# mengcaopku/DCNet

Measured on AMD Instinct MI355X. Metric: clips/sec (T=8, 416x416, bs8) fwd+bwd, higher is better.
Workload: dtype f32; 1 GPU; T=8 416x416 bs8/GPU L=20 fp32, 64 img/GPU/step as pairs, fwd+5 losses+bwd+RMSprop; arith=f16x2-split MFMA, fp32 accumulate, parallelism=dp1, ranks_seen=1, reducer=none, step=hipGraph replay (fwd+losses+bwd+RMSprop), sampler=mt

## Files before the change

dcnet_amd/csrc/coattn.h:

```cpp
#pragma once
#include <hip/hip_runtime.h>

int coattn_ld_pad(int hw);
bool coattn_on_gemm3(int b, int hw, int c);

struct CoOperand {
  const float* f; int ld; long long bs;
  const float* s; int lds; long long bss;
  const unsigned* amax;
};
inline CoOperand co_buffer(const float* p, int ld, long long bs, const unsigned* amax) { return CoOperand{p, ld, bs, p, ld, bs, amax}; }

struct CoProducts {
  int b, hw, c; hipStream_t stream; bool g3;
  CoProducts(int b_, int hw_, int c_, hipStream_t s) : b(b_), hw(hw_), c(c_), stream(s), g3(coattn_on_gemm3(b_, hw_, c_)) {}
  int nt(const CoOperand& A, const CoOperand& B, float* C, int ldc, long long c_bs, const float* row_scale, int accumulate,
         unsigned* amax_out = nullptr) const;
  int nn(const CoOperand& A, const CoOperand& B, float* C, int ldc, long long c_bs, const float* row_scale, int accumulate,
         unsigned* amax_out = nullptr) const;
  int tn(const CoOperand& A, const CoOperand& B, float* C, int ldc, long long c_bs, const float* row_scale, int accumulate,
         unsigned* amax_out = nullptr) const;
};

int coattn_amax_init_sets(unsigned* am, int sets, int slots, hipStream_t stream);
unsigned* coattn_ws_amax(float* ws, int b, int hw);
int coattn_amax_init(unsigned* am, hipStream_t stream);
int coattn_exp_sums(float* E, int nb, int hw, float temperature, float* rinv, float* cinv, float* ws, bool split, hipStream_t stream);
int coattn_rowdot_scale(const float* d, int ldd, long long bsd, const float* o, int ldo, long long bso, const float* inv, int b, int hw,
                        int c, float* delta, float* ds, unsigned* amax_d, unsigned* amax_ds, hipStream_t stream);
int coattn_da_bound(const unsigned* a1, const unsigned* a2, float temperature, unsigned* out, hipStream_t stream);
int coattn_dA(const float* E, float* dP1, const float* dP2, const float* rinv, const float* cinv, const float* d1, const float* d2,
              int b, int hw, float temperature, unsigned* amax_da, bool split, hipStream_t stream);
int coattn_fwd_operands(const CoOperand& F1, const CoOperand& F2, float* f1_attn, float* f2_attn, int ldo, long long bso, float* E,
                        float* rinv, float* cinv, float* ws, int b, int hw, int c, float temperature, hipStream_t stream);
```

dcnet_amd/csrc/coattn.hip:

```cpp
#include "igemm.h"
#include "prof.h"
#include "coattn.h"
#include "split4.h"

int tn_gemm_batched(const float* A, int lda, long long a_bs, const float* B, int ldb, long long b_bs,
                    float* C, int ldc, long long c_bs, const float* row_scale,
                    int M, int m_ld, int N, int K, int batch, int accumulate, hipStream_t stream,
                    const unsigned* amax_a = nullptr, const unsigned* amax_b = nullptr);

namespace {

constexpr int EXP_ROWS = 32;

template <bool SPLIT, bool COLS>
__global__ __launch_bounds__(256) void exp_sums_kernel(float* __restrict__ E, int hw, int ldE, float t,
                                                       float* __restrict__ rsum, float* __restrict__ colpart) {
  __shared__ float red[4][EXP_ROWS];
  const int b = blockIdx.y, rb = blockIdx.x;
  const int i0 = rb * EXP_ROWS;
  float* e = E + ((size_t)b * hw + i0) * ldE;
  float racc[EXP_ROWS];
#pragma unroll
  for (int r = 0; r < EXP_ROWS; ++r) racc[r] = 0.f;
  const int nrow = min(EXP_ROWS, hw - i0);
  for (int j = threadIdx.x * 4; j < ldE; j += 1024) {
    f32x4 v[EXP_ROWS];
#pragma unroll
    for (int r = 0; r < EXP_ROWS; ++r)
      v[r] = r < nrow ? *reinterpret_cast<const f32x4*>(e + (size_t)r * ldE + j) : f32x4{0.f, 0.f, 0.f, 0.f};
    f32x4 cs = {0.f, 0.f, 0.f, 0.f};
#pragma unroll
    for (int r = 0; r < EXP_ROWS; ++r) {
      if (r < nrow) {
        f32x4 o;
#pragma unroll
        for (int k = 0; k < 4; ++k) o[k] = (j + k < hw) ? expf(t * v[r][k] - t) : 0.f;
        if constexpr (SPLIT) split4_store(e + (size_t)r * ldE, j, o * SPLIT_SCALE_ONE);
        else *reinterpret_cast<f32x4*>(e + (size_t)r * ldE + j) = o;
        if constexpr (COLS) cs += o;
        racc[r] += (o[0] + o[1]) + (o[2] + o[3]);
      }
    }
    if constexpr (COLS) *reinterpret_cast<f32x4*>(colpart + ((size_t)rb * gridDim.y + b) * ldE + j) = cs;
  }
  const int lane = threadIdx.x & 63, wave = threadIdx.x >> 6;
#pragma unroll
  for (int r = 0; r < EXP_ROWS; ++r) {
    const float s = wave_sum(racc[r]);
    if (lane == 0) red[wave][r] = s;
  }
  __syncthreads();
  if (threadIdx.x < EXP_ROWS && i0 + threadIdx.x < hw)
    rsum[(size_t)b * hw + i0 + threadIdx.x] = 1.f / (red[0][threadIdx.x] + red[1][threadIdx.x] + red[2][threadIdx.x] + red[3][threadIdx.x]);
}

__global__ __launch_bounds__(256) void colsum_inv_kernel(const float* __restrict__ colpart, int nrb, int b, int hw, int ldE,
                                                         float* __restrict__ cinv) {
  const int j = blockIdx.x * 256 + threadIdx.x, bb = blockIdx.y;
  if (j >= hw) return;
  float s = 0.f;
  for (int rb = 0; rb < nrb; ++rb) s += colpart[((size_t)rb * b + bb) * ldE + j];
  cinv[(size_t)bb * hw + j] = 1.f / s;
}

enum { AM_ONE = 0, AM_DO1, AM_DO2, AM_DO1S, AM_DO2S, AM_DA, AM_DP1, AM_DP2, AM_SLOTS };
__global__ __launch_bounds__(256) void amax_init_kernel(unsigned* __restrict__ w, int total, int words_per_set) {
  for (int i = blockIdx.x * 256 + threadIdx.x; i < total; i += gridDim.x * 256)
    w[i] = (i % words_per_set) < DCN_AMAX_WORDS ? 0x3F800000u : 0u;
}

__global__ __launch_bounds__(256) void rowdot_scale_kernel(const float* __restrict__ d, int ldd, int64_t bsd,
                                                           const float* __restrict__ o, int ldo, int64_t bso, int hw,
                                                           const float* __restrict__ inv, int64_t rows, int c,
                                                           float* __restrict__ delta, float* __restrict__ ds,
                                                           unsigned* __restrict__ amax_d, unsigned* __restrict__ amax_ds) {
  __shared__ float red[4];
  const int lane = threadIdx.x & 63;
  const int64_t row = (int64_t)blockIdx.x * 4 + (threadIdx.x >> 6);
  float vmax = 0.f, s = 0.f;
  if (row < rows) {
    const int64_t bb = row / hw, i = row - bb * hw;
    s = inv[row];
    float acc = 0.f;
    for (int k = lane * 4; k < c; k += 256) {
      const f32x4 dv = *reinterpret_cast<const f32x4*>(d + bb * bsd + i * ldd + k);
      const f32x4 ov = *reinterpret_cast<const f32x4*>(o + bb * bso + i * ldo + k);
      acc += dv[0] * ov[0] + dv[1] * ov[1] + dv[2] * ov[2] + dv[3] * ov[3];
      *reinterpret_cast<f32x4*>(ds + row * c + k) = dv * s;
      vmax = fmaxf(fmaxf(vmax, fmaxf(fabsf(dv[0]), fabsf(dv[1]))), fmaxf(fabsf(dv[2]), fabsf(dv[3])));
    }
    acc = wave_sum(acc);
    if (lane == 0) delta[row] = acc;
  }
  const float vs = wave_max(vmax * s);
  amax_update_block(amax_d, vmax, red);
  __syncthreads();
  amax_update_block(amax_ds, vs, red);
}

template <bool ESPLIT, bool OSPLIT, bool COLS>
__global__ __launch_bounds__(256) void dA_kernel(const float* __restrict__ E, float* __restrict__ dP1, const float* __restrict__ dP2,
                                                 const float* __restrict__ rinv, const float* __restrict__ cinv,
                                                 const float* __restrict__ d1, const float* __restrict__ d2,
                                                 int hw, int ldE, float t, int64_t total4, unsigned* __restrict__ amax_da) {
  __shared__ float red[4];
  float vmax = 0.f;
  const int l4 = ldE >> 2;
  float s_out = 1.f;
  if constexpr (OSPLIT) s_out = split_pow2_scale(amax_read(amax_da));
  for (int64_t idx = (int64_t)blockIdx.x * 256 + threadIdx.x; idx < total4; idx += (int64_t)gridDim.x * 256) {
    const int64_t row = idx / l4;
    const int j = (int)(idx - row * l4) * 4;
    f32x4 e;
    if constexpr (ESPLIT) {
      const f32x4 hl = split4_load(E + row * ldE, j);
#pragma unroll
      for (int k = 0; k < 4; ++k) e[k] = hl[k] * (1.f / SPLIT_SCALE_ONE);
    } else {
      e = *reinterpret_cast<const f32x4*>(E + row * ldE + j);
    }
    const f32x4 p1 = *reinterpret_cast<const f32x4*>(dP1 + row * ldE + j);
    const float ri = rinv[row], di = d1[row];
    f32x4 o;
    if constexpr (COLS) {
      const int64_t bb = row / hw;
      const f32x4 p2 = *reinterpret_cast<const f32x4*>(dP2 + row * ldE + j);
#pragma unroll
      for (int k = 0; k < 4; ++k) {
        float v = 0.f;
        if (j + k < hw) v = t * e[k] * ((p1[k] - di) * ri + (p2[k] - d2[bb * hw + j + k]) * cinv[bb * hw + j + k]);
        o[k] = v;
      }
    } else {
      const float tr = t * ri;
#pragma unroll
      for (int k = 0; k < 4; ++k) o[k] = (j + k < hw) ? tr * e[k] * (p1[k] - di) : 0.f;
    }
    if constexpr (OSPLIT) {
      split4_store(dP1 + row * ldE, j, o * s_out);
    } else {
      *reinterpret_cast<f32x4*>(dP1 + row * ldE + j) = o;
      vmax = fmaxf(fmaxf(vmax, fmaxf(fabsf(o[0]), fabsf(o[1]))), fmaxf(fabsf(o[2]), fabsf(o[3])));
    }
  }
  if constexpr (!OSPLIT) amax_update_block(amax_da, vmax, red);
}

__global__ __launch_bounds__(64) void da_bound_kernel(const unsigned* __restrict__ a1, const unsigned* __restrict__ a2, float t,
                                                      unsigned* __restrict__ out) {
  const float b = 2.f * t * (__uint_as_float(amax_read(a1)) + (a2 ? __uint_as_float(amax_read(a2)) : 0.f));
  out[threadIdx.x & (DCN_AMAX_WORDS - 1)] = __float_as_uint(b);
}

inline int ld_pad(int hw) { return (hw + 31) / 32 * 32; }

void gemm_params(IgemmParams& p, const float* A, int lda, long long a_bs, const float* B, int ldb, long long b_bs,
                 float* C, int ldc, long long c_bs, int M, int N, int K, int batch) {
  p = IgemmParams{};
  p.osy = p.osx = p.isy = p.isx = 1; p.dense_out = 1;
  p.in = A; p.ldi = lda; p.in_bs = a_bs; p.wt = B; p.ldw = ldb; p.wt_bs = b_bs; p.out = C; p.ldo = ldc; p.out_bs = c_bs;
  p.ldr = ldc;
  p.N = 1; p.Hi = 1; p.Wi = M; p.Ho = 1; p.Wo = M; p.Hs = 1; p.Ws = M; p.M = M;
  p.Ci = K; p.Co = N; p.ntaps = 1; p.batch = batch;
}

}

static bool on_gemm3(int b, int hw, int c) { return c % 32 == 0 && gemm3_applicable(hw, c, hw, b) && gemm3_applicable(hw, hw, c, b); }

int coattn_ld_pad(int hw) { return ld_pad(hw); }
bool coattn_on_gemm3(int b, int hw, int c) { return on_gemm3(b, hw, c); }
unsigned* coattn_ws_amax(float* ws, int b, int hw) { return reinterpret_cast<unsigned*>(ws + (int64_t)cdiv(hw, EXP_ROWS) * b * ld_pad(hw)); }
int coattn_amax_init_sets(unsigned* am, int sets, int slots, hipStream_t stream) {
  const int total = sets * slots * DCN_AMAX_WORDS;
  hipLaunchKernelGGL(amax_init_kernel, dim3(cdiv(total, 256)), dim3(256), 0, stream, am, total, slots * DCN_AMAX_WORDS);
  DCN_CHECK_LAUNCH("coattn amax_init");
  return DCN_OK;
}
int coattn_amax_init(unsigned* am, hipStream_t stream) { return coattn_amax_init_sets(am, 1, AM_SLOTS, stream); }

int coattn_exp_sums(float* E, int nb, int hw, float temperature, float* rinv, float* cinv, float* ws, bool split, hipStream_t stream) {
  const int ldE = ld_pad(hw), nrb = cdiv(hw, EXP_ROWS);
  const auto kernel = split ? (cinv ? exp_sums_kernel<true, true> : exp_sums_kernel<true, false>)
                            : (cinv ? exp_sums_kernel<false, true> : exp_sums_kernel<false, false>);
  const int pid = prof_begin(12, (double)nb * hw * ldE * 8.0, stream);
  hipLaunchKernelGGL(kernel, dim3(nrb, nb), dim3(256), 0, stream, E, hw, ldE, temperature, rinv, ws);
  prof_end(pid, stream);
  DCN_CHECK_LAUNCH("exp_sums");
  if (!cinv) return DCN_OK;
  hipLaunchKernelGGL(colsum_inv_kernel, dim3(cdiv(hw, 256), nb), dim3(256), 0, stream, ws, nrb, nb, hw, ldE, cinv);
  DCN_CHECK_LAUNCH("colsum_inv");
  return DCN_OK;
}

int coattn_rowdot_scale(const float* d, int ldd, long long bsd, const float* o, int ldo, long long bso, const float* inv, int b, int hw,
                        int c, float* delta, float* ds, unsigned* amax_d, unsigned* amax_ds, hipStream_t stream) {
  const int64_t rows = (int64_t)b * hw;
  hipLaunchKernelGGL(rowdot_scale_kernel, dim3(cdiv(rows, 4)), dim3(256), 0, stream, d, ldd, (int64_t)bsd, o, ldo, (int64_t)bso, hw, inv, rows, c,
                     delta, ds, amax_d, amax_ds);
  DCN_CHECK_LAUNCH("rowdot_scale");
  return DCN_OK;
}

int coattn_da_bound(const unsigned* a1, const unsigned* a2, float temperature, unsigned* out, hipStream_t stream) {
  hipLaunchKernelGGL(da_bound_kernel, dim3(1), dim3(64), 0, stream, a1, a2, temperature, out);
  DCN_CHECK_LAUNCH("dA bound");
  return DCN_OK;
}

int coattn_dA(const float* E, float* dP1, const float* dP2, const float* rinv, const float* cinv, const float* d1, const float* d2,
              int b, int hw, float temperature, unsigned* amax_da, bool split, hipStream_t stream) {
  const int ldE = ld_pad(hw);
  const int64_t total4 = (int64_t)b * hw * (ldE / 4);
  int64_t g = (total4 + 255) / 256;
  if (g > 1024) g = 1024;
  const auto kernel = split ? (cinv ? dA_kernel<true, true, true> : dA_kernel<true, true, false>)
                            : (cinv ? dA_kernel<false, false, true> : dA_kernel<false, false, false>);
  const int pid = prof_begin(31, (double)total4 * 16.0 * (cinv ? 4.0 : 3.0), stream);
  hipLaunchKernelGGL(kernel, dim3((int)g), dim3(256), 0, stream, E, dP1, dP2, rinv, cinv, d1, d2, hw, ldE, temperature, total4, amax_da);
  prof_end(pid, stream);
  DCN_CHECK_LAUNCH("dA");
  return DCN_OK;
}

int CoProducts::nt(const CoOperand& A, const CoOperand& B, float* C, int ldc, long long c_bs, const float* row_scale, int accumulate,
                   unsigned* amax_out) const {
  if (g3) return gemm3_launch(A.s, A.lds, A.bss, 0, B.s, B.lds, B.bss, 0, C, ldc, c_bs, row_scale, row_scale ? hw : 0, hw, hw, c, b,
                              accumulate, A.amax, B.amax, stream, amax_out);
  IgemmParams p;
  gemm_params(p, A.f, A.ld, A.bs, B.f, B.ld, B.bs, C, ldc, c_bs, hw, hw, c, b);
  p.row_scale = row_scale; p.accumulate = accumulate; p.amax_a = A.amax; p.amax_b = B.amax;
  return igemm_launch(p, stream);
}
int CoProducts::nn(const CoOperand& A, const CoOperand& B, float* C, int ldc, long long c_bs, const float* row_scale, int accumulate,
                   unsigned* amax_out) const {
  if (g3) return gemm3_launch(A.s, A.lds, A.bss, 0, B.s, B.lds, B.bss, 1, C, ldc, c_bs, row_scale, row_scale ? hw : 0, hw, c, hw, b,
                              accumulate, A.amax, B.amax, stream, amax_out);
  IgemmParams p;
  gemm_params(p, A.f, A.ld, A.bs, B.f, B.ld, B.bs, C, ldc, c_bs, hw, c, A.ld, b);
  p.bmode = 1; p.kvalid = hw; p.row_scale = row_scale; p.accumulate = accumulate; p.amax_a = A.amax; p.amax_b = B.amax;
  return igemm_launch(p, stream);
}
int CoProducts::tn(const CoOperand& A, const CoOperand& B, float* C, int ldc, long long c_bs, const float* row_scale, int accumulate,
                   unsigned* amax_out) const {
  if (g3) return gemm3_launch(A.s, A.lds, A.bss, 1, B.s, B.lds, B.bss, 1, C, ldc, c_bs, row_scale, row_scale ? hw : 0, hw, c, hw, b,
                              accumulate, A.amax, B.amax, stream, amax_out);
  return tn_gemm_batched(A.f, A.ld, A.bs, B.f, B.ld, B.bs, C, ldc, c_bs, row_scale, hw, A.ld, c, hw, b, accumulate, stream, A.amax, B.amax);
}

int coattn_fwd_operands(const CoOperand& F1, const CoOperand& F2, float* f1_attn, float* f2_attn, int ldo, long long bso, float* E,
                        float* rinv, float* cinv, float* ws, int b, int hw, int c, float temperature, hipStream_t stream) {
  const CoProducts P(b, hw, c, stream);
  const int ldE = ld_pad(hw);
  const long long bsE = (long long)hw * ldE;
  const CoOperand Eo = co_buffer(E, ldE, bsE, F1.amax);
  int rc;
  if ((rc = P.nt(F1, F2, E, ldE, bsE, nullptr, 0))) return rc;
  if ((rc = coattn_exp_sums(E, b, hw, temperature, rinv, cinv, ws, P.g3, stream))) return rc;
  if ((rc = P.nn(Eo, F2, f1_attn, ldo, bso, rinv, 0))) return rc;
  if (f2_attn) rc = P.tn(Eo, F1, f2_attn, ldo, bso, cinv, 0);
  return rc;
}

extern "C" int64_t dcn_coattn_fwd_ws(int b, int hw, int c) {
  (void)c;
  return (int64_t)cdiv(hw, EXP_ROWS) * b * ld_pad(hw) + AM_SLOTS * DCN_AMAX_WORDS;
}
extern "C" int64_t dcn_coattn_e_size(int b, int hw) { return (int64_t)b * hw * ld_pad(hw); }
extern "C" int64_t dcn_coattn_saved_size(int b, int hw, int c) {
  return dcn_coattn_e_size(b, hw) + (on_gemm3(b, hw, c) ? (int64_t)2 * b * hw * c : 0);
}

extern "C" int dcn_coattn_fwd(const float* f1, const float* f2, int ldf, int64_t bsf, float* f1_attn, float* f2_attn, int ldo,
                              int64_t bso, float* E, float* rinv, float* cinv, float* ws,
                              int b, int hw, int c, float temperature, void* stream_) {
  hipStream_t stream = (hipStream_t)stream_;
  DCN_CHECK_ARG(f1 && f2 && f1_attn && E && rinv && cinv && ws, "coattn_fwd: null pointer");
  DCN_CHECK_ARG(b > 0 && hw > 0 && c > 0 && c % 32 == 0, "coattn_fwd: bad shape (c=%d must be a multiple of 32)", c);
  if (ldf <= 0) ldf = c;
  if (ldo <= 0) ldo = c;
  DCN_CHECK_ARG(ldf % 4 == 0 && ldo % 4 == 0, "coattn_fwd: ldf/ldo must be multiples of 4");
  if (bsf <= 0) bsf = (int64_t)hw * ldf;
  if (bso <= 0) bso = (int64_t)hw * ldo;
  DCN_CHECK_ARG(bsf % 4 == 0 && bso % 4 == 0, "coattn_fwd: batch strides must be multiples of 4");
  unsigned* am = coattn_ws_amax(ws, b, hw);
  int rc = coattn_amax_init(am, stream);
  if (rc) return rc;
  const unsigned* one = am + AM_ONE * DCN_AMAX_WORDS;
  float* f1s = E + dcn_coattn_e_size(b, hw);
  float* f2s = f1s + (int64_t)b * hw * c;
  const long long bss = (long long)hw * c;
  if (on_gemm3(b, hw, c)) {
    if ((rc = gemm3_presplit(f1, ldf, bsf, f1s, c, bss, b, hw, c, one, stream))) return rc;
    if ((rc = gemm3_presplit(f2, ldf, bsf, f2s, c, bss, b, hw, c, one, stream))) return rc;
  }
  return coattn_fwd_operands(CoOperand{f1, ldf, bsf, f1s, c, bss, one}, CoOperand{f2, ldf, bsf, f2s, c, bss, one}, f1_attn, f2_attn, ldo, bso,
                             E, rinv, cinv, ws, b, hw, c, temperature, stream);
}

extern "C" int64_t dcn_coattn_bwd_ws(int b, int hw, int c) {
  return (int64_t)2 * b * hw * ld_pad(hw) + (int64_t)2 * b * hw * c + (int64_t)2 * b * hw + AM_SLOTS * DCN_AMAX_WORDS +
         (on_gemm3(b, hw, c) ? (int64_t)2 * b * hw * c + 4 : 0);
}

extern "C" int dcn_coattn_bwd(const float* f1, const float* f2, int ldf, int64_t bsf,
                              const float* d_f1_attn, const float* d_f2_attn, int lddo, int64_t bsdo,
                              const float* f1_attn, const float* f2_attn, int ldo, int64_t bso,
                              const float* E, const float* rinv, const float* cinv,
                              float* d_f1, float* d_f2, int lddf, int64_t bsdf, int accumulate, float* ws,
                              int b, int hw, int c, float temperature, void* stream_) {
  hipStream_t stream = (hipStream_t)stream_;
  DCN_CHECK_ARG(f1 && f2 && d_f1_attn && d_f2_attn && f1_attn && f2_attn && E && rinv && cinv && d_f1 && d_f2 && ws,
                "coattn_bwd: null pointer");
  DCN_CHECK_ARG(b > 0 && hw > 0 && c > 0 && c % 32 == 0, "coattn_bwd: bad shape");
  if (ldf <= 0) ldf = c;
  if (ldo <= 0) ldo = c;
  if (lddo <= 0) lddo = c;
  if (lddf <= 0) lddf = c;
  if (bsf <= 0) bsf = (int64_t)hw * ldf;
  if (bso <= 0) bso = (int64_t)hw * ldo;
  if (bsdo <= 0) bsdo = (int64_t)hw * lddo;
  if (bsdf <= 0) bsdf = (int64_t)hw * lddf;
  const int ldE = ld_pad(hw);
  const long long rows = (long long)b * hw;
  float* dP1 = ws;
  float* dP2 = dP1 + rows * ldE;
  float* dO1s = dP2 + rows * ldE;
  float* dO2s = dO1s + rows * c;
  float* del1 = dO2s + rows * c;
  float* del2 = del1 + rows;
  unsigned* am = reinterpret_cast<unsigned*>(del2 + rows);
  int rc = coattn_amax_init(am, stream);
  if (rc) return rc;
  auto slot = [&](int i) { return am + i * DCN_AMAX_WORDS; };
  const CoProducts P(b, hw, c, stream);
  const long long bsE = (long long)hw * ldE, bss = (long long)hw * c;
  float* dO1p = reinterpret_cast<float*>(((uintptr_t)(am + AM_SLOTS * DCN_AMAX_WORDS) + 15) & ~(uintptr_t)15);
  float* dO2p = dO1p + rows * c;
  const float* f1s = E + dcn_coattn_e_size(b, hw);
  const float* f2s = f1s + rows * c;
  const CoOperand F1{f1, ldf, bsf, f1s, c, bss, slot(AM_ONE)}, F2{f2, ldf, bsf, f2s, c, bss, slot(AM_ONE)};
  const CoOperand DO1{d_f1_attn, lddo, bsdo, dO1p, c, bss, slot(AM_DO1)}, DO2{d_f2_attn, lddo, bsdo, dO2p, c, bss, slot(AM_DO2)};
  const CoOperand DO1S = co_buffer(dO1s, c, bss, slot(AM_DO1S)), DO2S = co_buffer(dO2s, c, bss, slot(AM_DO2S));
  const CoOperand Eo = co_buffer(E, ldE, bsE, slot(AM_ONE)), DA = co_buffer(dP1, ldE, bsE, slot(AM_DA));
  if ((rc = coattn_rowdot_scale(d_f1_attn, lddo, bsdo, f1_attn, ldo, bso, rinv, b, hw, c, del1, dO1s, slot(AM_DO1), slot(AM_DO1S), stream))) return rc;
  if ((rc = coattn_rowdot_scale(d_f2_attn, lddo, bsdo, f2_attn, ldo, bso, cinv, b, hw, c, del2, dO2s, slot(AM_DO2), slot(AM_DO2S), stream))) return rc;
  if (P.g3) {
    if ((rc = gemm3_presplit(d_f1_attn, lddo, bsdo, dO1p, c, bss, b, hw, c, slot(AM_DO1), stream))) return rc;
    if ((rc = gemm3_presplit(d_f2_attn, lddo, bsdo, dO2p, c, bss, b, hw, c, slot(AM_DO2), stream))) return rc;
    if ((rc = gemm3_presplit(dO1s, c, bss, dO1s, c, bss, b, hw, c, slot(AM_DO1S), stream))) return rc;
    if ((rc = gemm3_presplit(dO2s, c, bss, dO2s, c, bss, b, hw, c, slot(AM_DO2S), stream))) return rc;
  }
  if ((rc = P.nt(DO1, F2, dP1, ldE, bsE, nullptr, 0, slot(AM_DP1)))) return rc;
  if ((rc = P.nt(F1, DO2, dP2, ldE, bsE, nullptr, 0, slot(AM_DP2)))) return rc;
  if (P.g3 && (rc = coattn_da_bound(slot(AM_DP1), slot(AM_DP2), temperature, slot(AM_DA), stream))) return rc;
  if ((rc = coattn_dA(E, dP1, dP2, rinv, cinv, del1, del2, b, hw, temperature, slot(AM_DA), P.g3, stream))) return rc;
  if ((rc = P.nn(DA, F2, d_f1, lddf, bsdf, nullptr, accumulate))) return rc;
  if ((rc = P.nn(Eo, DO2S, d_f1, lddf, bsdf, nullptr, 1))) return rc;
  if ((rc = P.tn(DA, F1, d_f2, lddf, bsdf, nullptr, accumulate))) return rc;
  return P.tn(Eo, DO1S, d_f2, lddf, bsdf, nullptr, 1);
}
```

dcnet_amd/csrc/coattn_center.hip:

```cpp
#include "igemm.h"
#include "coattn.h"

namespace {

enum { AM_ONE = 0, AM_DO, AM_DOS, AM_DP, AM_DA, AM_SLOTS };

inline int frame_of(int n, int ctr) { return n < ctr ? n : n + 1; }

int check_shape(const char* who, int b, int t, int hw, int c, int ctr) {
  DCN_CHECK_ARG(b > 0 && hw > 0 && c > 0 && c % 32 == 0, "%s: bad shape (b=%d hw=%d; c=%d must be a multiple of 32)", who, b, hw, c);
  DCN_CHECK_ARG(t >= 2, "%s: a window needs t >= 2 frames (t=%d)", who, t);
  DCN_CHECK_ARG(ctr >= 0 && ctr < t, "%s: ctr=%d out of range [0, %d)", who, ctr, t);
  return DCN_OK;
}

}

extern "C" int64_t dcn_coattn_center_saved_size(int b, int t, int hw, int c) {
  if (b <= 0 || t < 2 || hw <= 0 || c <= 0) return 0;
  return dcn_coattn_e_size(b * (t - 1), hw) + (coattn_on_gemm3(b, hw, c) ? (int64_t)b * t * hw * c : 0);
}
extern "C" int64_t dcn_coattn_center_fwd_ws(int b, int t, int hw, int c) {
  (void)b; (void)t; (void)hw; (void)c;
  return AM_SLOTS * DCN_AMAX_WORDS;
}

extern "C" int dcn_coattn_center_fwd(const float* clips, float* attn, int ldo, int64_t bso, int64_t nso, float* E, float* rinv, float* ws,
                                     int b, int t, int hw, int c, int ctr, float temperature, void* stream_) {
  hipStream_t stream = (hipStream_t)stream_;
  DCN_CHECK_ARG(clips && attn && E && rinv && ws, "coattn_center_fwd: null pointer");
  int rc = check_shape("coattn_center_fwd", b, t, hw, c, ctr);
  if (rc) return rc;
  if (ldo <= 0) ldo = c;
  if (bso <= 0) bso = (int64_t)hw * ldo;
  if (nso <= 0) nso = (int64_t)b * bso;
  DCN_CHECK_ARG(ldo >= c && ldo % 4 == 0 && bso % 4 == 0 && nso % 4 == 0 && ((uintptr_t)attn & 15) == 0 && ((uintptr_t)clips & 15) == 0,
                "coattn_center_fwd: ldo >= c; ldo, the strides (floats) multiples of 4; 16-byte aligned tensors");
  const int ldE = coattn_ld_pad(hw), nn = t - 1;
  const long long bsE = (long long)hw * ldE, bsf = (long long)t * hw * c, frame = (long long)hw * c;
  const CoProducts P(b, hw, c, stream);
  unsigned* am = reinterpret_cast<unsigned*>(ws);
  if ((rc = coattn_amax_init_sets(am, 1, AM_SLOTS, stream))) return rc;
  const unsigned* one = am + AM_ONE * DCN_AMAX_WORDS;
  float* clips_s = E + dcn_coattn_e_size(b * nn, hw);
  auto frame_op = [&](int f) { return CoOperand{clips + f * frame, c, bsf, clips_s + f * frame, c, bsf, one}; };
  if (P.g3 && (rc = gemm3_presplit(clips, c, frame, clips_s, c, frame, b * t, hw, c, one, stream))) return rc;
  for (int n = 0; n < nn; ++n)
    if ((rc = P.nt(frame_op(ctr), frame_op(frame_of(n, ctr)), E + (int64_t)n * b * bsE, ldE, bsE, nullptr, 0))) return rc;
  if ((rc = coattn_exp_sums(E, b * nn, hw, temperature, rinv, nullptr, nullptr, P.g3, stream))) return rc;
  for (int n = 0; n < nn; ++n) {
    const CoOperand En = co_buffer(E + (int64_t)n * b * bsE, ldE, bsE, one);
    if ((rc = P.nn(En, frame_op(frame_of(n, ctr)), attn + n * nso, ldo, bso, rinv + (int64_t)n * b * hw, 0))) return rc;
  }
  return DCN_OK;
}

extern "C" int64_t dcn_coattn_center_bwd_ws(int b, int t, int hw, int c) {
  if (b <= 0 || t < 2 || hw <= 0 || c <= 0) return 0;
  const int64_t rows = (int64_t)b * hw;
  return rows * coattn_ld_pad(hw) + rows * c + rows + (int64_t)(t - 1) * AM_SLOTS * DCN_AMAX_WORDS + (coattn_on_gemm3(b, hw, c) ? rows * c + 4 : 0);
}

extern "C" int dcn_coattn_center_bwd(const float* clips, const float* d_attn, int lddo, int64_t bsdo, int64_t nsdo,
                                     const float* attn, int ldo, int64_t bso, int64_t nso, const float* E, const float* rinv,
                                     float* d_clips, int accumulate, float* ws,
                                     int b, int t, int hw, int c, int ctr, float temperature, void* stream_) {
  hipStream_t stream = (hipStream_t)stream_;
  DCN_CHECK_ARG(clips && d_attn && attn && E && rinv && d_clips && ws, "coattn_center_bwd: null pointer");
  int rc = check_shape("coattn_center_bwd", b, t, hw, c, ctr);
  if (rc) return rc;
  if (ldo <= 0) ldo = c;
  if (lddo <= 0) lddo = c;
  if (bso <= 0) bso = (int64_t)hw * ldo;
  if (bsdo <= 0) bsdo = (int64_t)hw * lddo;
  if (nso <= 0) nso = (int64_t)b * bso;
  if (nsdo <= 0) nsdo = (int64_t)b * bsdo;
  DCN_CHECK_ARG(ldo >= c && lddo >= c && ldo % 4 == 0 && lddo % 4 == 0 && bso % 4 == 0 && bsdo % 4 == 0 && nso % 4 == 0 && nsdo % 4 == 0 &&
                    (((uintptr_t)attn | (uintptr_t)d_attn | (uintptr_t)clips | (uintptr_t)d_clips | (uintptr_t)ws) & 15) == 0,
                "coattn_center_bwd: ldo, lddo >= c; row / batch / neighbour strides (floats) multiples of 4; 16-byte aligned tensors");
  const int ldE = coattn_ld_pad(hw), nn = t - 1;
  const long long rows = (long long)b * hw;
  const long long bsE = (long long)hw * ldE, bsf = (long long)t * hw * c, frame = (long long)hw * c;
  const CoProducts P(b, hw, c, stream);
  float* dP = ws;
  float* dOs = dP + rows * ldE;
  float* del = dOs + rows * c;
  unsigned* am = reinterpret_cast<unsigned*>(del + rows);
  float* dOp = reinterpret_cast<float*>(((uintptr_t)(am + (size_t)nn * AM_SLOTS * DCN_AMAX_WORDS) + 15) & ~(uintptr_t)15);
  if ((rc = coattn_amax_init_sets(am, nn, AM_SLOTS, stream))) return rc;
  const float* clips_s = E + dcn_coattn_e_size(b * nn, hw);
  for (int n = 0; n < nn; ++n) {
    const long long fj = frame_of(n, ctr) * frame, fc = ctr * frame;
    const float* rn = rinv + (int64_t)n * rows;
    const float* dO = d_attn + n * nsdo;
    unsigned* amn = am + (size_t)n * AM_SLOTS * DCN_AMAX_WORDS;
    auto slot = [&](int i) { return amn + i * DCN_AMAX_WORDS; };
    const CoOperand Fj{clips + fj, c, bsf, clips_s + fj, c, bsf, slot(AM_ONE)}, Fc{clips + fc, c, bsf, clips_s + fc, c, bsf, slot(AM_ONE)};
    const CoOperand DO{dO, lddo, bsdo, dOp, c, frame, slot(AM_DO)}, DOS = co_buffer(dOs, c, frame, slot(AM_DOS));
    const CoOperand En = co_buffer(E + (int64_t)n * b * bsE, ldE, bsE, slot(AM_ONE)), DA = co_buffer(dP, ldE, bsE, slot(AM_DA));
    if ((rc = coattn_rowdot_scale(dO, lddo, bsdo, attn + n * nso, ldo, bso, rn, b, hw, c, del, dOs, slot(AM_DO), slot(AM_DOS), stream))) return rc;
    if (P.g3) {
      if ((rc = gemm3_presplit(dO, lddo, bsdo, dOp, c, frame, b, hw, c, slot(AM_DO), stream))) return rc;
      if ((rc = gemm3_presplit(dOs, c, frame, dOs, c, frame, b, hw, c, slot(AM_DOS), stream))) return rc;
    }
    if ((rc = P.nt(DO, Fj, dP, ldE, bsE, nullptr, 0, slot(AM_DP)))) return rc;
    if (P.g3 && (rc = coattn_da_bound(slot(AM_DP), nullptr, temperature, slot(AM_DA), stream))) return rc;
    if ((rc = coattn_dA(En.f, dP, nullptr, rn, nullptr, del, nullptr, b, hw, temperature, slot(AM_DA), P.g3, stream))) return rc;
    if ((rc = P.nn(DA, Fj, d_clips + fc, c, bsf, nullptr, (n > 0 || accumulate) ? 1 : 0))) return rc;
    if ((rc = P.tn(DA, Fc, d_clips + fj, c, bsf, nullptr, 0))) return rc;
    if ((rc = P.tn(En, DOS, d_clips + fj, c, bsf, nullptr, 1))) return rc;
  }
  return DCN_OK;
}
```

dcnet_amd/csrc/gemm3.hip:

```cpp
#include "igemm.h"
#include "prof.h"
#include "split4.h"

namespace {

typedef _Float16 f16x8_t __attribute__((ext_vector_type(8)));
typedef short s16x4 __attribute__((ext_vector_type(4)));
typedef short s16x8 __attribute__((ext_vector_type(8)));
typedef __attribute__((address_space(3))) void lds_void;

#ifndef G3_ABL
#define G3_ABL 0
#endif
constexpr unsigned G3_OOB = 0x80000000u;
constexpr int G3_BM = 256, G3_BN = 256, G3_STAGES = 4;
constexpr int G3_TILE = 256 * 64;
constexpr int G3_STAGE = 2 * G3_TILE;
constexpr int G3_LDS = G3_STAGES * G3_STAGE;

struct G3Params {
  const float* A; const float* B; float* C;
  long long a_bs, b_bs, c_bs;
  int lda, ldb, ldc;
  int M, N, K;
  int a_rows, b_rows;
  int a_cols, b_cols;
  int tiles_m, tiles_n;
  const float* row_scale; long long rs_bs;
  int accumulate;
  const unsigned* amax_a; const unsigned* amax_b;
  unsigned* amax_out;
  int var;
  int abl;
};

__device__ __forceinline__ int g3_tswz(int krow) { return (krow & 1) | ((krow & 2) << 1); }

template <bool AT, bool BT, bool H1 = false>
__global__ __launch_bounds__(512, 1) void gemm3_kernel(const G3Params p) {
  extern __shared__ __attribute__((aligned(1024))) unsigned char smem3g[];
  const int tid = threadIdx.x, lane = tid & 63;
  const int wave = __builtin_amdgcn_readfirstlane(tid >> 6);
  const int wm = wave >> 2, wn = wave & 3;
  const int per_batch = p.tiles_m * p.tiles_n;
  const int lin = xcd_remap(blockIdx.x, gridDim.x);
  const int batch = __builtin_amdgcn_readfirstlane(lin / per_batch), t_ = lin - batch * per_batch;
  const int bm = __builtin_amdgcn_readfirstlane(t_ / p.tiles_n), bn = t_ - bm * p.tiles_n;
  const int m0 = bm * G3_BM, n0 = bn * G3_BN;
  const int kslices = (p.K + 15) >> 4;

  const float* a_base = p.A + batch * p.a_bs + (AT ? 0 : (long long)m0 * p.lda);
  const float* b_base = p.B + batch * p.b_bs + (BT ? 0 : (long long)n0 * p.ldb);
  const int a_rows_left = AT ? p.a_rows : p.a_rows - m0, b_rows_left = BT ? p.b_rows : p.b_rows - n0;
  const long long a_bytes = ((long long)(a_rows_left - 1) * p.lda + p.a_cols) * 4, b_bytes = ((long long)(b_rows_left - 1) * p.ldb + p.b_cols) * 4;
  const __amdgpu_buffer_rsrc_t a_rs = __builtin_amdgcn_make_buffer_rsrc((void*)a_base, 0, a_bytes > 0x7FFFFFF0LL ? 0x7FFFFFF0 : (int)a_bytes, 0x00020000);
  const __amdgpu_buffer_rsrc_t b_rs = __builtin_amdgcn_make_buffer_rsrc((void*)b_base, 0, b_bytes > 0x7FFFFFF0LL ? 0x7FFFFFF0 : (int)b_bytes, 0x00020000);

  unsigned voff[4];
  int sstep_a, sstep_b;
#pragma unroll
  for (int e = 0; e < 2; ++e) {
    const int j = 2 * wave + e;
    if (AT) {
      voff[e] = (unsigned)((long long)j * p.lda * 4 + m0 * 4 + ((lane ^ g3_tswz(j)) << 4));
      if (m0 + ((lane ^ g3_tswz(j)) << 2) >= p.a_cols) voff[e] = G3_OOB;
    } else {
      const int row = 16 * j + (lane >> 2), c = (lane & 3) ^ ((row >> 2) & 3);
      voff[e] = row < a_rows_left ? (unsigned)((long long)row * p.lda * 4 + c * 16) : G3_OOB;
    }
    if (BT) {
      voff[2 + e] = (unsigned)((long long)j * p.ldb * 4 + n0 * 4 + ((lane ^ g3_tswz(j)) << 4));
      if (n0 + ((lane ^ g3_tswz(j)) << 2) >= p.b_cols) voff[2 + e] = G3_OOB;
    } else {
      const int row = 16 * j + (lane >> 2), c = (lane & 3) ^ ((row >> 2) & 3);
      voff[2 + e] = row < b_rows_left ? (unsigned)((long long)row * p.ldb * 4 + c * 16) : G3_OOB;
    }
  }
  sstep_a = AT ? 16 * p.lda * 4 : 64;
  sstep_b = BT ? 16 * p.ldb * 4 : 64;
  const int my_dst = 2 * wave * 1024;

  int k_done = 0;
  auto issue_a = [&]() {
    const bool live = k_done < kslices && !(G3_ABL && (p.abl & 1));
    unsigned char* st = smem3g + (k_done & (G3_STAGES - 1)) * G3_STAGE + my_dst;
    int sa_ = live ? k_done * sstep_a : 0;
    if (G3_ABL && (p.abl & 8)) sa_ = 0;
#pragma unroll
    for (int e = 0; e < 2; ++e)
      __builtin_amdgcn_raw_ptr_buffer_load_lds(a_rs, (lds_void*)(st + e * 1024), 16, (int)(live ? voff[e] : G3_OOB), sa_, 0, 0);
  };
  auto issue_b = [&]() {
    const bool live = k_done < kslices && !(G3_ABL && (p.abl & 1));
    unsigned char* st = smem3g + (k_done & (G3_STAGES - 1)) * G3_STAGE + my_dst;
    int sb_ = live ? k_done * sstep_b : 0;
    if (G3_ABL && (p.abl & 8)) sb_ = 0;
#pragma unroll
    for (int e = 0; e < 2; ++e)
      __builtin_amdgcn_raw_ptr_buffer_load_lds(b_rs, (lds_void*)(st + G3_TILE + e * 1024), 16, (int)(live ? voff[2 + e] : G3_OOB), sb_, 0, 0);
    ++k_done;
  };
  auto issue = [&]() { issue_a(); issue_b(); };

  const int g = lane >> 5;
  const int hh = lane >> 5, gg = (lane >> 4) & 1, qq = (lane & 15) >> 2, pp = lane & 3;
  int a_rd[4][2], b_rd[2][2];
#pragma unroll
  for (int mi = 0; mi < 4; ++mi) {
    if (AT) {
      const int c = wm * 128 + mi * 32 + 16 * gg + 4 * pp;
#pragma unroll
      for (int r2 = 0; r2 < 2; ++r2) {
        const int kr = 8 * hh + 4 * r2 + qq;
        a_rd[mi][r2] = kr * 1024 + ((((c >> 3) * 2) ^ g3_tswz(kr)) << 4) + (c & 7) * 2;
      }
    } else {
      const int ar = wm * 128 + mi * 32 + (lane & 31);
      a_rd[mi][0] = ar * 64 + (((2 * g) ^ ((ar >> 2) & 3)) << 4);
      a_rd[mi][1] = ar * 64 + (((2 * g + 1) ^ ((ar >> 2) & 3)) << 4);
    }
  }
#pragma unroll
  for (int ni = 0; ni < 2; ++ni) {
    if (BT) {
      const int c = wn * 64 + ni * 32 + 16 * gg + 4 * pp;
#pragma unroll
      for (int r2 = 0; r2 < 2; ++r2) {
        const int kr = 8 * hh + 4 * r2 + qq;
        b_rd[ni][r2] = G3_TILE + kr * 1024 + ((((c >> 3) * 2) ^ g3_tswz(kr)) << 4) + (c & 7) * 2;
      }
    } else {
      const int br = wn * 64 + ni * 32 + (lane & 31);
      b_rd[ni][0] = G3_TILE + br * 64 + (((2 * g) ^ ((br >> 2) & 3)) << 4);
      b_rd[ni][1] = G3_TILE + br * 64 + (((2 * g + 1) ^ ((br >> 2) & 3)) << 4);
    }
  }
  auto tr_read = [&](const unsigned char* ptr) {
    return __builtin_amdgcn_ds_read_tr16_b64_v4i16((__attribute__((address_space(3))) s16x4*)(ptr));
  };
  auto tfrag = [&](const unsigned char* st, int off0, int off1, int plane) {
    const s16x4 lo = tr_read(st + (off0 ^ (plane << 4))), hi = tr_read(st + (off1 ^ (plane << 4)));
    const s16x8 v = {lo[0], lo[1], lo[2], lo[3], hi[0], hi[1], hi[2], hi[3]};
    return __builtin_bit_cast(f16x8_t, v);
  };

  f32x16 acc[4][2];
#pragma unroll
  for (int mi = 0; mi < 4; ++mi)
#pragma unroll
    for (int ni = 0; ni < 2; ++ni)
#pragma unroll
      for (int r = 0; r < 16; ++r) acc[mi][ni][r] = 0.f;

  for (int s = 0; s < G3_STAGES - 1; ++s) issue();

  asm volatile("s_waitcnt vmcnt(%0)" :: "n"((G3_STAGES - 2) * 4) : "memory");
  if (wm == 1) __builtin_amdgcn_s_barrier();
  for (int it = 0; it < kslices; ++it) {
    __builtin_amdgcn_s_barrier();
    asm volatile("" ::: "memory");
    const unsigned char* st = smem3g + (it & (G3_STAGES - 1)) * G3_STAGE;
    f16x8_t bh[2], bl[2];
    f16x8_t ah[4], al[4];
    if (G3_ABL && (p.abl & 2)) {
#pragma unroll
      for (int ni = 0; ni < 2; ++ni) { bh[ni] = f16x8_t{(_Float16)it, 0, 0, 0, 0, 0, 0, 0}; bl[ni] = bh[ni]; }
#pragma unroll
      for (int mi = 0; mi < 4; ++mi) { ah[mi] = bh[0]; al[mi] = bh[1]; }
    } else {
#pragma unroll
      for (int ni = 0; ni < 2; ++ni) {
        if (BT) { bh[ni] = tfrag(st, b_rd[ni][0], b_rd[ni][1], 0); if constexpr (!H1) bl[ni] = tfrag(st, b_rd[ni][0], b_rd[ni][1], 1); }
        else { bh[ni] = *reinterpret_cast<const f16x8_t*>(st + b_rd[ni][0]); if constexpr (!H1) bl[ni] = *reinterpret_cast<const f16x8_t*>(st + b_rd[ni][1]); }
      }
#pragma unroll
      for (int mi = 0; mi < 4; ++mi) {
        if (AT) { ah[mi] = tfrag(st, a_rd[mi][0], a_rd[mi][1], 0); if constexpr (!H1) al[mi] = tfrag(st, a_rd[mi][0], a_rd[mi][1], 1); }
        else { ah[mi] = *reinterpret_cast<const f16x8_t*>(st + a_rd[mi][0]); if constexpr (!H1) al[mi] = *reinterpret_cast<const f16x8_t*>(st + a_rd[mi][1]); }
      }
    }
    if (p.var >= 1) {
      issue_a();
      if (wm == 1) asm volatile("s_waitcnt vmcnt(%0)" :: "n"((G3_STAGES - 2) * 4 - 2) : "memory");
    } else {
      issue();
      if (wm == 1) asm volatile("s_waitcnt vmcnt(%0)" :: "n"((G3_STAGES - 2) * 4) : "memory");
    }
    asm volatile("s_waitcnt lgkmcnt(0)" ::: "memory");
    __builtin_amdgcn_s_barrier();
    asm volatile("" ::: "memory");
    if (G3_ABL && (p.abl & 4)) {
#pragma unroll
      for (int mi = 0; mi < 4; ++mi) { asm volatile("" :: "v"(ah[mi]), "v"(al[mi])); }
#pragma unroll
      for (int ni = 0; ni < 2; ++ni) { asm volatile("" :: "v"(bh[ni]), "v"(bl[ni])); }
    } else {
      __builtin_amdgcn_s_setprio(1);
      if constexpr (!H1) {
#pragma unroll
        for (int mi = 0; mi < 4; ++mi)
#pragma unroll
          for (int ni = 0; ni < 2; ++ni) acc[mi][ni] = __builtin_amdgcn_mfma_f32_32x32x16_f16(al[mi], bh[ni], acc[mi][ni], 0, 0, 0);
        if (p.var == 2) issue_b();
#pragma unroll
        for (int mi = 0; mi < 4; ++mi)
#pragma unroll
          for (int ni = 0; ni < 2; ++ni) acc[mi][ni] = __builtin_amdgcn_mfma_f32_32x32x16_f16(ah[mi], bl[ni], acc[mi][ni], 0, 0, 0);
      } else if (p.var == 2) issue_b();
#pragma unroll
      for (int mi = 0; mi < 4; ++mi)
#pragma unroll
        for (int ni = 0; ni < 2; ++ni) acc[mi][ni] = __builtin_amdgcn_mfma_f32_32x32x16_f16(ah[mi], bh[ni], acc[mi][ni], 0, 0, 0);
      __builtin_amdgcn_s_setprio(0);
    }
    if (p.var == 1) issue_b();
    if (wm == 0) asm volatile("s_waitcnt vmcnt(%0)" :: "n"((G3_STAGES - 2) * 4) : "memory");
  }
  if (wm == 0) __builtin_amdgcn_s_barrier();
  asm volatile("s_waitcnt vmcnt(0)" ::: "memory");

  const float dq = 1.f / (split_pow2_scale(amax_read(p.amax_a)) * split_pow2_scale(amax_read(p.amax_b)));
  float* __restrict__ cb = p.C + batch * p.c_bs;
  const float* rs = p.row_scale ? p.row_scale + batch * p.rs_bs : nullptr;
  float vmax = 0.f;
#pragma unroll
  for (int mi = 0; mi < 4; ++mi)
#pragma unroll
    for (int r = 0; r < 16; ++r) {
      const int m = m0 + wm * 128 + mi * 32 + 4 * g + (r & 3) + 8 * (r >> 2);
      if (m >= p.M) continue;
      const float f = rs ? dq * rs[m] : dq;
#pragma unroll
      for (int ni = 0; ni < 2; ++ni) {
        const int n = n0 + wn * 64 + ni * 32 + (lane & 31);
        if (n >= p.N) continue;
        float v = acc[mi][ni][r] * f;
        float* dst = cb + (long long)m * p.ldc + n;
        if (p.accumulate) v += *dst;
        *dst = v;
        vmax = fmaxf(vmax, fabsf(v));
      }
    }
  if (p.amax_out) {
    vmax = wave_max(vmax);
    if (lane == 0) amax_update(p.amax_out, vmax, blockIdx.x * 8 + wave);
  }
}

__global__ __launch_bounds__(256) void presplit_kernel(const float* __restrict__ src, int ld, long long bs, float* __restrict__ dst, int ldd,
                                                        long long bsd, int rows, int c, long long total8, const unsigned* __restrict__ amax) {
  const float s = split_pow2_scale(amax_read(amax));
  const int c8 = c >> 3;
  for (long long i = (long long)blockIdx.x * 256 + threadIdx.x; i < total8; i += (long long)gridDim.x * 256) {
    const long long row_all = i / c8; const int o = (int)(i - row_all * c8);
    const long long b = row_all / rows; const int row = (int)(row_all - b * rows);
    const float* sp = src + b * bs + (long long)row * ld + o * 8;
    const f32x4 x0 = *reinterpret_cast<const f32x4*>(sp) * s, x1 = *reinterpret_cast<const f32x4*>(sp + 4) * s;
    f16x8_t h, l;
#pragma unroll
    for (int e = 0; e < 4; ++e) { h[e] = (_Float16)x0[e]; h[4 + e] = (_Float16)x1[e]; }
#pragma unroll
    for (int e = 0; e < 4; ++e) { l[e] = (_Float16)(x0[e] - (float)h[e]); l[4 + e] = (_Float16)(x1[e] - (float)h[4 + e]); }
    float* dp = dst + b * bsd + (long long)row * ldd + o * 8;
    *reinterpret_cast<f16x8_t*>(dp) = h;
    *reinterpret_cast<f16x8_t*>(dp + 4) = l;
  }
}

DCN_KNOB(g_gemm3, "Gemm3", 1, "gemm3.hip: the co-attention products on pre-split operands (0 = implicit-GEMM / weight-gradient tiles; + 256 * v = schedule variant v; + 16 * bits = timing ablations, results WRONG)",
         nullptr, "-DG3_ABL=1", G3_ABL != 0, [](int v) { return (v & 0xF0) != 0; });
DCN_KNOB(g_gemm3_h1, "H1gemm3", 1, "gemm3.hip: one f16 piece per operand in the bf16 precision modes (0 = both pieces, fp32-accurate co-attention)");

template <bool AT, bool BT, bool H1>
int launch3g_(const G3Params& p, int grid, hipStream_t stream) {
  static DcnPerDeviceFlag attr_once;
  if (attr_once.first()) {
    (void)hipFuncSetAttribute(reinterpret_cast<const void*>(&gemm3_kernel<AT, BT, H1>), hipFuncAttributeMaxDynamicSharedMemorySize, G3_LDS);
  }
  hipLaunchKernelGGL((gemm3_kernel<AT, BT, H1>), dim3(grid), dim3(512), G3_LDS, stream, p);
  return DCN_OK;
}
template <bool AT, bool BT>
int launch3g(const G3Params& p, int grid, hipStream_t stream) {
  if (g_gemm3_h1 && igemm_precision() == 2) return launch3g_<AT, BT, true>(p, grid, stream);
  return launch3g_<AT, BT, false>(p, grid, stream);
}

}

int gemm3_variant() { const int v = g_gemm3 >> 8; return (v == 1 || v == 2) ? v : 0; }
extern "C" int dcn_gemm3_variant() { return gemm3_variant(); }

bool gemm3_applicable(int M, int N, int K, int batch) {
  return g_gemm3 && (igemm_precision() == 4 || igemm_precision() == 2) && M >= 512 && N >= 256 && K >= 64 && batch >= 1;
}

int gemm3_presplit(const float* src, int ld, long long bs, float* dst, int ldd, long long bsd, int batch, int rows, int c,
                   const unsigned* amax, hipStream_t stream) {
  DCN_CHECK_ARG(src && dst && amax && c % 8 == 0 && ld % 4 == 0 && ldd % 4 == 0 && bs % 4 == 0 && bsd % 4 == 0, "gemm3_presplit: bad argument");
  const long long total8 = (long long)batch * rows * (c / 8);
  long long g = (total8 + 255) / 256; if (g > 16384) g = 16384;
  hipLaunchKernelGGL(presplit_kernel, dim3((int)g), dim3(256), 0, stream, src, ld, bs, dst, ldd, bsd, rows, c, total8, amax);
  DCN_CHECK_LAUNCH("gemm3_presplit");
  return DCN_OK;
}

int gemm3_launch(const float* A, int lda, long long a_bs, int at, const float* B, int ldb, long long b_bs, int bt,
                 float* C, int ldc, long long c_bs, const float* row_scale, long long rs_bs,
                 int M, int N, int K, int batch, int accumulate, const unsigned* amax_a, const unsigned* amax_b, hipStream_t stream,
                 unsigned* amax_out) {
  DCN_CHECK_ARG(A && B && C && amax_a && amax_b, "gemm3: null pointer");
  DCN_CHECK_ARG(lda % 4 == 0 && ldb % 4 == 0 && a_bs % 4 == 0 && b_bs % 4 == 0 && (((uintptr_t)A | (uintptr_t)B) & 15) == 0, "gemm3: 16-byte rows");
  G3Params p{};
  p.A = A; p.B = B; p.C = C; p.a_bs = a_bs; p.b_bs = b_bs; p.c_bs = c_bs; p.lda = lda; p.ldb = ldb; p.ldc = ldc;
  p.M = M; p.N = N; p.K = K;
  const int k16 = (K + 15) / 16 * 16;
  p.a_rows = at ? K : M; p.b_rows = bt ? K : N;
  p.a_cols = at ? (M + 7) / 8 * 8 : k16; p.b_cols = bt ? (N + 7) / 8 * 8 : k16;
  DCN_CHECK_ARG(p.a_cols <= lda && p.b_cols <= ldb, "gemm3: rows shorter than the tile reads (lda=%d ldb=%d)", lda, ldb);
  p.tiles_m = cdiv(M, G3_BM); p.tiles_n = cdiv(N, G3_BN);
  p.row_scale = row_scale; p.rs_bs = rs_bs; p.accumulate = accumulate; p.amax_a = amax_a; p.amax_b = amax_b; p.amax_out = amax_out; p.abl = (g_gemm3 >> 4) & 15; p.var = gemm3_variant();
  const int grid = p.tiles_m * p.tiles_n * batch;
  const int pid = prof_begin(40, 2.0 * batch * (double)M * N * K, stream);
  int rc;
  if (at) rc = bt ? launch3g<true, true>(p, grid, stream) : DCN_ERR_ARG;
  else rc = bt ? launch3g<false, true>(p, grid, stream) : launch3g<false, false>(p, grid, stream);
  prof_end(pid, stream);
  DCN_CHECK_ARG(rc == DCN_OK, "gemm3: no A^T . B^T form");
  DCN_CHECK_LAUNCH("gemm3");
  return DCN_OK;
}

extern "C" int dcn_gemm3_supported(int m, int n, int k, int batch) { return gemm3_applicable(m, n, k, batch) ? 1 : 0; }

extern "C" int dcn_gemm3_presplit(const float* src, int ld, int64_t bs, float* dst, int ldd, int64_t bsd, int batch, int rows, int c,
                                  const uint32_t* amax, void* stream) {
  return gemm3_presplit(src, ld, bs, dst, ldd, bsd, batch, rows, c, amax, (hipStream_t)stream);
}

extern "C" int dcn_gemm3(const float* a, int lda, int64_t a_bs, int a_t, const float* b, int ldb, int64_t b_bs, int b_t,
                         float* c, int ldc, int64_t c_bs, const float* row_scale, int64_t rs_bs,
                         int m, int n, int k, int batch, int accumulate, const uint32_t* amax_a, const uint32_t* amax_b, void* stream) {
  DCN_CHECK_ARG(m > 0 && n > 0 && k > 0 && batch > 0, "gemm3: empty problem");
  return gemm3_launch(a, lda, a_bs, a_t, b, ldb, b_bs, b_t, c, ldc, c_bs, row_scale, rs_bs, m, n, k, batch, accumulate, amax_a, amax_b,
                      (hipStream_t)stream, nullptr);
}
```

dcnet_amd/csrc/igemm.h:

```cpp
#pragma once
#include "common.h"

#define IGEMM_MAX_TAPS 16


struct IgemmParams {
  const float* in;
  const float* wt;
  const float* f8;
  const unsigned* amax_a;
  const unsigned* amax_b;
  const void* wt16;
  const float* b_scale;
  unsigned* amax_out;
  float* out;
  const float* scale;
  const float* shift;
  const float* residual;
  float* stats;
  const float* row_scale;
  int batch;
  long long in_bs, wt_bs, out_bs;
  int bmode;
  int kvalid;
  int N, Hi, Wi, Ci, ldi;
  int Ho, Wo;
  int Hs, Ws;
  int oy0, ox0, osy, osx;
  int isy, isx;
  int Co, ldo, ldr, ldw;
  int M;
  int ntaps;
  int cpt, kiters;
  int act; float slope;
  int accumulate, dense_out, c4;
  int acc_post;
  int tap_dy[IGEMM_MAX_TAPS], tap_dx[IGEMM_MAX_TAPS], tap_w[IGEMM_MAX_TAPS];
  int ncls;
  int cls_M[4], cls_Hs[4], cls_Ws[4], cls_oy0[4], cls_ox0[4], cls_ntaps[4];
  const float* bt_y; const float* bt_mean; const float* bt_invstd; const float* bt_gamma; const float* bt_beta;
  int bt_act; float bt_slope;
  const unsigned char* a_scale8; const unsigned char* b_scale8;
};
inline double epilogue_reads(const IgemmParams& p) { return 1.0 + (p.accumulate ? 1.0 : 0.0) + (p.residual ? 1.0 : 0.0) + (p.bt_y ? 1.0 : 0.0); }
bool igemm_tap_capable(const IgemmParams& p);

int igemm_grid_m(int M, int Co, int ntaps);
int igemm_launch(const IgemmParams& p, hipStream_t stream);
bool igemm_will_presplit(long long rows, int Co, int ntaps, int Ci);

bool conv3_applicable(const IgemmParams& p, int precision, int gran);
int conv3_launch(const IgemmParams& p, int gran, hipStream_t stream);
bool conv3x_takes(const IgemmParams& p, int gran);
int conv3x_launch(const IgemmParams& p, int gran, hipStream_t stream);
int conv3b_bm(int M, int Co, int Wi);
bool conv3b_takes(const IgemmParams& p);
int conv3b_launch(const IgemmParams& p, int out_f32, hipStream_t stream);

bool conv1_applicable(const IgemmParams& p, int precision, int gran);
int conv1_launch(const IgemmParams& p, int gran, hipStream_t stream);
int conv1_tile_of(long long rows, int Co, int ntaps, int Ci, int stats, int gran, int storage16);
int conv1b_grid_m(int M, int Co, int ntaps, int s1_w = 0);
int conv1b_launch(const IgemmParams& p, int out_f32, hipStream_t stream);
int conv1q_grid_m(int M, int Co);
int conv1q_launch(const IgemmParams& p, int out_f32, hipStream_t stream);
bool conv2b_takes(int M, int Co, int ntaps);
int conv2b_launch(const IgemmParams& p, int out_f32, hipStream_t stream);


bool stem_applicable(const IgemmParams& p, const float* scratch);
int stem_launch(const IgemmParams& p, float* scratch, hipStream_t stream);

bool dgrad2_applicable(int n, int h, int wd, int cin, int cout, int ksize, int stride, int accumulate);
struct DcnBnTap { const float* y; const float* mean; const float* invstd; const float* gamma; const float* beta; int act; float slope;
                  float* stats; int stats_rows; };
int nconv1_launch_b16(int mode, const void* x, int ldi, const void* w16, void* y, int ldo, float* stats, int stats_rows,
                      int n, int h, int wd, int stride, hipStream_t stream);
int dgrad2_launch_b16(const void* dy, int lddy, const void* wt16, void* dx, int n, int h, int wd, int cin, int accumulate, hipStream_t stream);
int dgrad2_grid(int n, int h, int wd, int cin);
int dgrad2_launch(const float* dy, int lddy, const float* wt, float* dx, int n, int h, int wd, int cin, int accumulate,
                  const uint32_t* amax_dy, const uint32_t* amax_w, const DcnBnTap* tap, hipStream_t stream);
bool gemm3_applicable(int M, int N, int K, int batch);
int gemm3_presplit(const float* src, int ld, long long bs, float* dst, int ldd, long long bsd, int batch, int rows, int c,
                   const unsigned* amax, hipStream_t stream);
int gemm3_launch(const float* A, int lda, long long a_bs, int at, const float* B, int ldb, long long b_bs, int bt,
                 float* C, int ldc, long long c_bs, const float* row_scale, long long rs_bs,
                 int M, int N, int K, int batch, int accumulate, const unsigned* amax_a, const unsigned* amax_b, hipStream_t stream,
                 unsigned* amax_out = nullptr);
int igemm_precision();
extern int g_abl;
extern int g_wsplit;
struct DcnPreAct { const float* scale; const float* shift; int act; float slope; };
bool nconv1_applicable(int mode, int n, int h, int wd, int cin, int cout, int ksize, int stride);
int nconv1_launch(int mode, const float* x, int ldi, const float* w, float* y, int ldo, float* stats, int stats_rows,
                  int n, int h, int wd, int stride, const uint32_t* amax_x, const uint32_t* amax_w, const DcnPreAct* pre, hipStream_t stream);
```

Baseline: 88.12 clips/s.

## Fuse co-attention exp/softmax sums and dA into gemm3 product epilogues

Adds fused epilogues to the gemm3 co-attention kernel. In the forward pass the exponentials and per-tile row/column partial sums are computed inside the NT product, so the separate exp_sums pass over E is gone. In the backward pass the dA computation is done in the epilogue of the second dP product, which removes the dP2 buffer round trip and the standalone dA kernel; a norm of dO2 bounds the split scale in place of dP2's amax. The costs are heavier epilogues (LDS reductions, extra loads of E, rinv, cinv and the deltas), swapped MFMA operand order, a norm-based scale bound that may be looser, and small colsum kernels.

```diff
diff --git a/dcnet_amd/csrc/coattn.h b/dcnet_amd/csrc/coattn.h
--- a/dcnet_amd/csrc/coattn.h
+++ b/dcnet_amd/csrc/coattn.h
@@ -13,21 +13,26 @@
 
 struct CoProducts {
   int b, hw, c; hipStream_t stream; bool g3;
-  CoProducts(int b_, int hw_, int c_, hipStream_t s) : b(b_), hw(hw_), c(c_), stream(s), g3(coattn_on_gemm3(b_, hw_, c_)) {}
+  bool fused;
+  CoProducts(int b_, int hw_, int c_, hipStream_t s);
   int nt(const CoOperand& A, const CoOperand& B, float* C, int ldc, long long c_bs, const float* row_scale, int accumulate,
          unsigned* amax_out = nullptr) const;
   int nn(const CoOperand& A, const CoOperand& B, float* C, int ldc, long long c_bs, const float* row_scale, int accumulate,
          unsigned* amax_out = nullptr) const;
   int tn(const CoOperand& A, const CoOperand& B, float* C, int ldc, long long c_bs, const float* row_scale, int accumulate,
          unsigned* amax_out = nullptr) const;
+  int nt_exp(const CoOperand& A, const CoOperand& B, float* E, float temperature, float* rinv, float* cinv, float* ws) const;
+  int nt_dA(const CoOperand& A, const CoOperand& B, float* dP1, const float* E, const float* rinv, const float* cinv, const float* d1,
+            const float* d2, float temperature, const unsigned* amax_da) const;
 };
+int64_t coattn_exp_ws(int b, int hw, bool cols);
 
 int coattn_amax_init_sets(unsigned* am, int sets, int slots, hipStream_t stream);
 unsigned* coattn_ws_amax(float* ws, int b, int hw);
 int coattn_amax_init(unsigned* am, hipStream_t stream);
 int coattn_exp_sums(float* E, int nb, int hw, float temperature, float* rinv, float* cinv, float* ws, bool split, hipStream_t stream);
 int coattn_rowdot_scale(const float* d, int ldd, long long bsd, const float* o, int ldo, long long bso, const float* inv, int b, int hw,
-                        int c, float* delta, float* ds, unsigned* amax_d, unsigned* amax_ds, hipStream_t stream);
+                        int c, float* delta, float* ds, unsigned* amax_d, unsigned* amax_ds, hipStream_t stream, unsigned* norm_d = nullptr);
 int coattn_da_bound(const unsigned* a1, const unsigned* a2, float temperature, unsigned* out, hipStream_t stream);
 int coattn_dA(const float* E, float* dP1, const float* dP2, const float* rinv, const float* cinv, const float* d1, const float* d2,
               int b, int hw, float temperature, unsigned* amax_da, bool split, hipStream_t stream);
diff --git a/dcnet_amd/csrc/coattn.hip b/dcnet_amd/csrc/coattn.hip
--- a/dcnet_amd/csrc/coattn.hip
+++ b/dcnet_amd/csrc/coattn.hip
@@ -63,21 +63,23 @@
   cinv[(size_t)bb * hw + j] = 1.f / s;
 }
 
-enum { AM_ONE = 0, AM_DO1, AM_DO2, AM_DO1S, AM_DO2S, AM_DA, AM_DP1, AM_DP2, AM_SLOTS };
+enum { AM_ONE = 0, AM_DO1, AM_DO2, AM_DO1S, AM_DO2S, AM_DA, AM_DP1, AM_DP2, AM_NDO2, AM_SLOTS };
 __global__ __launch_bounds__(256) void amax_init_kernel(unsigned* __restrict__ w, int total, int words_per_set) {
   for (int i = blockIdx.x * 256 + threadIdx.x; i < total; i += gridDim.x * 256)
     w[i] = (i % words_per_set) < DCN_AMAX_WORDS ? 0x3F800000u : 0u;
 }
 
+template <bool NORM>
 __global__ __launch_bounds__(256) void rowdot_scale_kernel(const float* __restrict__ d, int ldd, int64_t bsd,
                                                            const float* __restrict__ o, int ldo, int64_t bso, int hw,
                                                            const float* __restrict__ inv, int64_t rows, int c,
                                                            float* __restrict__ delta, float* __restrict__ ds,
-                                                           unsigned* __restrict__ amax_d, unsigned* __restrict__ amax_ds) {
+                                                           unsigned* __restrict__ amax_d, unsigned* __restrict__ amax_ds,
+                                                           unsigned* __restrict__ norm_d) {
   __shared__ float red[4];
   const int lane = threadIdx.x & 63;
   const int64_t row = (int64_t)blockIdx.x * 4 + (threadIdx.x >> 6);
-  float vmax = 0.f, s = 0.f;
+  float vmax = 0.f, s = 0.f, sq = 0.f;
   if (row < rows) {
     const int64_t bb = row / hw, i = row - bb * hw;
     s = inv[row];
@@ -91,11 +93,22 @@
     }
     acc = wave_sum(acc);
     if (lane == 0) delta[row] = acc;
+    if constexpr (NORM) {
+      for (int k = lane * 4; k < c; k += 256) {
+        const f32x4 dv = *reinterpret_cast<const f32x4*>(d + bb * bsd + i * ldd + k);
+        sq += dv[0] * dv[0] + dv[1] * dv[1] + dv[2] * dv[2] + dv[3] * dv[3];
+      }
+    }
   }
   const float vs = wave_max(vmax * s);
   amax_update_block(amax_d, vmax, red);
   __syncthreads();
   amax_update_block(amax_ds, vs, red);
+  if constexpr (NORM) {
+    const float nrm = sqrtf(wave_sum(sq)) * 1.0009765625f;
+    __syncthreads();
+    amax_update_block(norm_d, nrm, red);
+  }
 }
 
 template <bool ESPLIT, bool OSPLIT, bool COLS>
@@ -170,6 +183,8 @@
 
 int coattn_ld_pad(int hw) { return ld_pad(hw); }
 bool coattn_on_gemm3(int b, int hw, int c) { return on_gemm3(b, hw, c); }
+CoProducts::CoProducts(int b_, int hw_, int c_, hipStream_t s)
+    : b(b_), hw(hw_), c(c_), stream(s), g3(on_gemm3(b_, hw_, c_)), fused(g3 && gemm3_fused()) {}
 unsigned* coattn_ws_amax(float* ws, int b, int hw) { return reinterpret_cast<unsigned*>(ws + (int64_t)cdiv(hw, EXP_ROWS) * b * ld_pad(hw)); }
 int coattn_amax_init_sets(unsigned* am, int sets, int slots, hipStream_t stream) {
   const int total = sets * slots * DCN_AMAX_WORDS;
@@ -194,10 +209,10 @@
 }
 
 int coattn_rowdot_scale(const float* d, int ldd, long long bsd, const float* o, int ldo, long long bso, const float* inv, int b, int hw,
-                        int c, float* delta, float* ds, unsigned* amax_d, unsigned* amax_ds, hipStream_t stream) {
+                        int c, float* delta, float* ds, unsigned* amax_d, unsigned* amax_ds, hipStream_t stream, unsigned* norm_d) {
   const int64_t rows = (int64_t)b * hw;
-  hipLaunchKernelGGL(rowdot_scale_kernel, dim3(cdiv(rows, 4)), dim3(256), 0, stream, d, ldd, (int64_t)bsd, o, ldo, (int64_t)bso, hw, inv, rows, c,
-                     delta, ds, amax_d, amax_ds);
+  hipLaunchKernelGGL(norm_d ? rowdot_scale_kernel<true> : rowdot_scale_kernel<false>, dim3(cdiv(rows, 4)), dim3(256), 0, stream, d, ldd, (int64_t)bsd,
+                     o, ldo, (int64_t)bso, hw, inv, rows, c, delta, ds, amax_d, amax_ds, norm_d);
   DCN_CHECK_LAUNCH("rowdot_scale");
   return DCN_OK;
 }
@@ -248,6 +263,31 @@
   return tn_gemm_batched(A.f, A.ld, A.bs, B.f, B.ld, B.bs, C, ldc, c_bs, row_scale, hw, A.ld, c, hw, b, accumulate, stream, A.amax, B.amax);
 }
 
+int64_t coattn_exp_ws(int b, int hw, bool cols) {
+  const int64_t tiles = cdiv(hw, 256);
+  return (tiles * b * hw + 3) / 4 * 4 + (cols ? tiles * b * ld_pad(hw) : 0);
+}
+int CoProducts::nt_exp(const CoOperand& A, const CoOperand& B, float* E, float temperature, float* rinv, float* cinv, float* ws) const {
+  DCN_CHECK_ARG(fused && ws && (((uintptr_t)ws) & 15) == 0, "coattn: the exp epilogue needs gemm3.hip's fused launches and an aligned workspace");
+  const int ldE = ld_pad(hw), tiles = cdiv(hw, 256);
+  float* rowpart = ws;
+  float* colpart = cinv ? ws + coattn_exp_ws(b, hw, false) : nullptr;
+  int rc = gemm3_launch_exp(A.s, A.lds, A.bss, B.s, B.lds, B.bss, E, ldE, (long long)hw * ldE, hw, hw, c, b, A.amax, B.amax, temperature,
+                            rowpart, colpart, stream);
+  if (rc) return rc;
+  hipLaunchKernelGGL(colsum_inv_kernel, dim3(cdiv(hw, 256), b), dim3(256), 0, stream, rowpart, tiles, b, hw, hw, rinv);
+  if (cinv) hipLaunchKernelGGL(colsum_inv_kernel, dim3(cdiv(hw, 256), b), dim3(256), 0, stream, colpart, tiles, b, hw, ldE, cinv);
+  DCN_CHECK_LAUNCH("tile sums -> rinv, cinv");
+  return DCN_OK;
+}
+int CoProducts::nt_dA(const CoOperand& A, const CoOperand& B, float* dP1, const float* E, const float* rinv, const float* cinv,
+                      const float* d1, const float* d2, float temperature, const unsigned* amax_da) const {
+  DCN_CHECK_ARG(fused, "coattn: the dA epilogue needs gemm3.hip's fused launches");
+  const int ldE = ld_pad(hw);
+  return gemm3_launch_dA(A.s, A.lds, A.bss, B.s, B.lds, B.bss, dP1, ldE, (long long)hw * ldE, hw, hw, c, b, A.amax, B.amax, temperature, E,
+                         rinv, cinv, d1, d2, amax_da, stream);
+}
+
 int coattn_fwd_operands(const CoOperand& F1, const CoOperand& F2, float* f1_attn, float* f2_attn, int ldo, long long bso, float* E,
                         float* rinv, float* cinv, float* ws, int b, int hw, int c, float temperature, hipStream_t stream) {
   const CoProducts P(b, hw, c, stream);
@@ -255,8 +295,12 @@
   const long long bsE = (long long)hw * ldE;
   const CoOperand Eo = co_buffer(E, ldE, bsE, F1.amax);
   int rc;
-  if ((rc = P.nt(F1, F2, E, ldE, bsE, nullptr, 0))) return rc;
-  if ((rc = coattn_exp_sums(E, b, hw, temperature, rinv, cinv, ws, P.g3, stream))) return rc;
+  if (P.fused) {
+    if ((rc = P.nt_exp(F1, F2, E, temperature, rinv, cinv, ws))) return rc;
+  } else {
+    if ((rc = P.nt(F1, F2, E, ldE, bsE, nullptr, 0))) return rc;
+    if ((rc = coattn_exp_sums(E, b, hw, temperature, rinv, cinv, ws, P.g3, stream))) return rc;
+  }
   if ((rc = P.nn(Eo, F2, f1_attn, ldo, bso, rinv, 0))) return rc;
   if (f2_attn) rc = P.tn(Eo, F1, f2_attn, ldo, bso, cinv, 0);
   return rc;
@@ -344,7 +388,8 @@
   const CoOperand DO1S = co_buffer(dO1s, c, bss, slot(AM_DO1S)), DO2S = co_buffer(dO2s, c, bss, slot(AM_DO2S));
   const CoOperand Eo = co_buffer(E, ldE, bsE, slot(AM_ONE)), DA = co_buffer(dP1, ldE, bsE, slot(AM_DA));
   if ((rc = coattn_rowdot_scale(d_f1_attn, lddo, bsdo, f1_attn, ldo, bso, rinv, b, hw, c, del1, dO1s, slot(AM_DO1), slot(AM_DO1S), stream))) return rc;
-  if ((rc = coattn_rowdot_scale(d_f2_attn, lddo, bsdo, f2_attn, ldo, bso, cinv, b, hw, c, del2, dO2s, slot(AM_DO2), slot(AM_DO2S), stream))) return rc;
+  if ((rc = coattn_rowdot_scale(d_f2_attn, lddo, bsdo, f2_attn, ldo, bso, cinv, b, hw, c, del2, dO2s, slot(AM_DO2), slot(AM_DO2S), stream,
+                                P.fused ? slot(AM_NDO2) : nullptr))) return rc;
   if (P.g3) {
     if ((rc = gemm3_presplit(d_f1_attn, lddo, bsdo, dO1p, c, bss, b, hw, c, slot(AM_DO1), stream))) return rc;
     if ((rc = gemm3_presplit(d_f2_attn, lddo, bsdo, dO2p, c, bss, b, hw, c, slot(AM_DO2), stream))) return rc;
@@ -352,9 +397,11 @@
     if ((rc = gemm3_presplit(dO2s, c, bss, dO2s, c, bss, b, hw, c, slot(AM_DO2S), stream))) return rc;
   }
   if ((rc = P.nt(DO1, F2, dP1, ldE, bsE, nullptr, 0, slot(AM_DP1)))) return rc;
-  if ((rc = P.nt(F1, DO2, dP2, ldE, bsE, nullptr, 0, slot(AM_DP2)))) return rc;
-  if (P.g3 && (rc = coattn_da_bound(slot(AM_DP1), slot(AM_DP2), temperature, slot(AM_DA), stream))) return rc;
-  if ((rc = coattn_dA(E, dP1, dP2, rinv, cinv, del1, del2, b, hw, temperature, slot(AM_DA), P.g3, stream))) return rc;
+  if (!P.fused && (rc = P.nt(F1, DO2, dP2, ldE, bsE, nullptr, 0, slot(AM_DP2)))) return rc;
+  if (P.g3 && (rc = coattn_da_bound(slot(AM_DP1), slot(P.fused ? AM_NDO2 : AM_DP2), temperature, slot(AM_DA), stream))) return rc;
+  if (P.fused) rc = P.nt_dA(F1, DO2, dP1, E, rinv, cinv, del1, del2, temperature, slot(AM_DA));
+  else rc = coattn_dA(E, dP1, dP2, rinv, cinv, del1, del2, b, hw, temperature, slot(AM_DA), P.g3, stream);
+  if (rc) return rc;
   if ((rc = P.nn(DA, F2, d_f1, lddf, bsdf, nullptr, accumulate))) return rc;
   if ((rc = P.nn(Eo, DO2S, d_f1, lddf, bsdf, nullptr, 1))) return rc;
   if ((rc = P.tn(DA, F1, d_f2, lddf, bsdf, nullptr, accumulate))) return rc;
diff --git a/dcnet_amd/csrc/coattn_center.hip b/dcnet_amd/csrc/coattn_center.hip
--- a/dcnet_amd/csrc/coattn_center.hip
+++ b/dcnet_amd/csrc/coattn_center.hip
@@ -21,8 +21,8 @@
   return dcn_coattn_e_size(b * (t - 1), hw) + (coattn_on_gemm3(b, hw, c) ? (int64_t)b * t * hw * c : 0);
 }
 extern "C" int64_t dcn_coattn_center_fwd_ws(int b, int t, int hw, int c) {
-  (void)b; (void)t; (void)hw; (void)c;
-  return AM_SLOTS * DCN_AMAX_WORDS;
+  (void)t;
+  return AM_SLOTS * DCN_AMAX_WORDS + (coattn_on_gemm3(b, hw, c) ? coattn_exp_ws(b, hw, false) : 0);
 }
 
 extern "C" int dcn_coattn_center_fwd(const float* clips, float* attn, int ldo, int64_t bso, int64_t nso, float* E, float* rinv, float* ws,
@@ -45,9 +45,13 @@
   float* clips_s = E + dcn_coattn_e_size(b * nn, hw);
   auto frame_op = [&](int f) { return CoOperand{clips + f * frame, c, bsf, clips_s + f * frame, c, bsf, one}; };
   if (P.g3 && (rc = gemm3_presplit(clips, c, frame, clips_s, c, frame, b * t, hw, c, one, stream))) return rc;
-  for (int n = 0; n < nn; ++n)
-    if ((rc = P.nt(frame_op(ctr), frame_op(frame_of(n, ctr)), E + (int64_t)n * b * bsE, ldE, bsE, nullptr, 0))) return rc;
-  if ((rc = coattn_exp_sums(E, b * nn, hw, temperature, rinv, nullptr, nullptr, P.g3, stream))) return rc;
+  for (int n = 0; n < nn; ++n) {
+    if (P.fused) rc = P.nt_exp(frame_op(ctr), frame_op(frame_of(n, ctr)), E + (int64_t)n * b * bsE, temperature, rinv + (int64_t)n * b * hw, nullptr,
+                               ws + AM_SLOTS * DCN_AMAX_WORDS);
+    else rc = P.nt(frame_op(ctr), frame_op(frame_of(n, ctr)), E + (int64_t)n * b * bsE, ldE, bsE, nullptr, 0);
+    if (rc) return rc;
+  }
+  if (!P.fused && (rc = coattn_exp_sums(E, b * nn, hw, temperature, rinv, nullptr, nullptr, P.g3, stream))) return rc;
   for (int n = 0; n < nn; ++n) {
     const CoOperand En = co_buffer(E + (int64_t)n * b * bsE, ldE, bsE, one);
     if ((rc = P.nn(En, frame_op(frame_of(n, ctr)), attn + n * nso, ldo, bso, rinv + (int64_t)n * b * hw, 0))) return rc;
diff --git a/dcnet_amd/csrc/gemm3.hip b/dcnet_amd/csrc/gemm3.hip
--- a/dcnet_amd/csrc/gemm3.hip
+++ b/dcnet_amd/csrc/gemm3.hip
@@ -32,12 +32,20 @@
   unsigned* amax_out;
   int var;
   int abl;
+  float t;
+  float* rowpart; float* colpart;
+  const float* E;
+  const float* rinv; const float* cinv; const float* d1; const float* d2;
+  const unsigned* amax_da;
 };
+constexpr int G3_COLLD = 260;
 
 __device__ __forceinline__ int g3_tswz(int krow) { return (krow & 1) | ((krow & 2) << 1); }
 
-template <bool AT, bool BT, bool H1 = false>
+enum { G3_EPI_NONE = 0, G3_EPI_EXP = 1, G3_EPI_EXP_ROWS = 2, G3_EPI_DA = 3 };
+template <bool AT, bool BT, bool H1 = false, int EPI = G3_EPI_NONE>
 __global__ __launch_bounds__(512, 1) void gemm3_kernel(const G3Params p) {
+  static_assert(EPI == G3_EPI_NONE || (!AT && !BT && !H1), "the fused epilogues exist for the two-piece NT form");
   extern __shared__ __attribute__((aligned(1024))) unsigned char smem3g[];
   const int tid = threadIdx.x, lane = tid & 63;
   const int wave = __builtin_amdgcn_readfirstlane(tid >> 6);
@@ -151,6 +159,10 @@
     for (int ni = 0; ni < 2; ++ni)
 #pragma unroll
       for (int r = 0; r < 16; ++r) acc[mi][ni][r] = 0.f;
+  auto mma = [](const f16x8_t& a, const f16x8_t& b, const f32x16& c) {
+    if constexpr (EPI != G3_EPI_NONE) return __builtin_amdgcn_mfma_f32_32x32x16_f16(b, a, c, 0, 0, 0);
+    else return __builtin_amdgcn_mfma_f32_32x32x16_f16(a, b, c, 0, 0, 0);
+  };
 
   for (int s = 0; s < G3_STAGES - 1; ++s) issue();
 
@@ -200,17 +212,17 @@
 #pragma unroll
         for (int mi = 0; mi < 4; ++mi)
 #pragma unroll
-          for (int ni = 0; ni < 2; ++ni) acc[mi][ni] = __builtin_amdgcn_mfma_f32_32x32x16_f16(al[mi], bh[ni], acc[mi][ni], 0, 0, 0);
+          for (int ni = 0; ni < 2; ++ni) acc[mi][ni] = mma(al[mi], bh[ni], acc[mi][ni]);
         if (p.var == 2) issue_b();
 #pragma unroll
         for (int mi = 0; mi < 4; ++mi)
 #pragma unroll
-          for (int ni = 0; ni < 2; ++ni) acc[mi][ni] = __builtin_amdgcn_mfma_f32_32x32x16_f16(ah[mi], bl[ni], acc[mi][ni], 0, 0, 0);
+          for (int ni = 0; ni < 2; ++ni) acc[mi][ni] = mma(ah[mi], bl[ni], acc[mi][ni]);
       } else if (p.var == 2) issue_b();
 #pragma unroll
       for (int mi = 0; mi < 4; ++mi)
 #pragma unroll
-        for (int ni = 0; ni < 2; ++ni) acc[mi][ni] = __builtin_amdgcn_mfma_f32_32x32x16_f16(ah[mi], bh[ni], acc[mi][ni], 0, 0, 0);
+        for (int ni = 0; ni < 2; ++ni) acc[mi][ni] = mma(ah[mi], bh[ni], acc[mi][ni]);
       __builtin_amdgcn_s_setprio(0);
     }
     if (p.var == 1) issue_b();
@@ -218,6 +230,119 @@
   }
   if (wm == 0) __builtin_amdgcn_s_barrier();
   asm volatile("s_waitcnt vmcnt(0)" ::: "memory");
+
+  if constexpr (EPI == G3_EPI_EXP || EPI == G3_EPI_EXP_ROWS) {
+    __builtin_amdgcn_s_barrier();
+    asm volatile("" ::: "memory");
+    float* rowbuf = reinterpret_cast<float*>(smem3g);
+    float* colbuf = rowbuf + 8 * 256;
+    float* colred = colbuf + 64 * G3_COLLD;
+    const int nb = gridDim.x / per_batch;
+    const float dq = 1.f / (split_pow2_scale(amax_read(p.amax_a)) * split_pow2_scale(amax_read(p.amax_b)));
+    const float t = p.t;
+    float* __restrict__ cb = p.C + batch * p.c_bs;
+    f32x4 csum[2][4];
+#pragma unroll
+    for (int ni = 0; ni < 2; ++ni)
+#pragma unroll
+      for (int q = 0; q < 4; ++q) csum[ni][q] = f32x4{0.f, 0.f, 0.f, 0.f};
+#pragma unroll
+    for (int mi = 0; mi < 4; ++mi) {
+      const int ml = wm * 128 + mi * 32 + (lane & 31), m = m0 + ml;
+      const bool mok = m < p.M;
+      float* crow = cb + (long long)m * p.ldc;
+      float rs = 0.f;
+#pragma unroll
+      for (int ni = 0; ni < 2; ++ni)
+#pragma unroll
+        for (int q = 0; q < 4; ++q) {
+          const int n = n0 + wn * 64 + ni * 32 + 8 * q + 4 * g;
+          f32x4 o;
+#pragma unroll
+          for (int k = 0; k < 4; ++k) {
+            const float a = acc[mi][ni][4 * q + k] * dq;
+            o[k] = (mok && n + k < p.N) ? expf(t * a - t) : 0.f;
+          }
+          if (mok && n < p.ldc) split4_store(crow, n, o * SPLIT_SCALE_ONE);
+          rs += (o[0] + o[1]) + (o[2] + o[3]);
+          if constexpr (EPI == G3_EPI_EXP) csum[ni][q] += o;
+        }
+      rowbuf[(wn * 2 + g) * 256 + ml] = rs;
+    }
+    if constexpr (EPI == G3_EPI_EXP) {
+#pragma unroll
+      for (int ni = 0; ni < 2; ++ni)
+#pragma unroll
+        for (int q = 0; q < 4; ++q)
+          *reinterpret_cast<f32x4*>(colbuf + (wm * 32 + (lane & 31)) * G3_COLLD + wn * 64 + ni * 32 + 8 * q + 4 * g) = csum[ni][q];
+    }
+    __syncthreads();
+    if (tid < 256) {
+      float s = 0.f;
+#pragma unroll
+      for (int w = 0; w < 8; ++w) s += rowbuf[w * 256 + tid];
+      if (m0 + tid < p.M) p.rowpart[((long long)bn * nb + batch) * p.M + m0 + tid] = s;
+    }
+    if constexpr (EPI == G3_EPI_EXP) {
+      const int c = tid & 255, w = tid >> 8;
+      float s = 0.f;
+#pragma unroll 8
+      for (int r = 0; r < 32; ++r) s += colbuf[(w * 32 + r) * G3_COLLD + c];
+      if (w == 1) colred[c] = s;
+      __syncthreads();
+      if (w == 0 && n0 + c < p.ldc) p.colpart[((long long)bm * nb + batch) * p.ldc + n0 + c] = s + colred[c];
+    }
+    return;
+  }
+  if constexpr (EPI == G3_EPI_DA) {
+    const float dq = 1.f / (split_pow2_scale(amax_read(p.amax_a)) * split_pow2_scale(amax_read(p.amax_b)));
+    const float s_out = split_pow2_scale(amax_read(p.amax_da));
+    const float t = p.t;
+    float* __restrict__ cb = p.C + batch * p.c_bs;
+    const float* __restrict__ eb = p.E + batch * p.c_bs;
+    __builtin_amdgcn_s_barrier();
+    asm volatile("" ::: "memory");
+    float* cvec = reinterpret_cast<float*>(smem3g);
+    if (tid < 256) {
+      const bool ok = n0 + tid < p.N;
+      cvec[tid] = ok ? p.cinv[(long long)batch * p.N + n0 + tid] : 0.f;
+      cvec[256 + tid] = ok ? p.d2[(long long)batch * p.N + n0 + tid] : 0.f;
+    }
+    __syncthreads();
+#pragma unroll
+    for (int mi = 0; mi < 4; ++mi) {
+      const int m = m0 + wm * 128 + mi * 32 + (lane & 31);
+      if (m >= p.M) continue;
+      const float ri = p.rinv[(long long)batch * p.M + m], di = p.d1[(long long)batch * p.M + m];
+      float* crow = cb + (long long)m * p.ldc;
+      const float* erow = eb + (long long)m * p.ldc;
+#pragma unroll
+      for (int ni = 0; ni < 2; ++ni) {
+        f32x4 p1[4], e[4];
+#pragma unroll
+        for (int q = 0; q < 4; ++q) {
+          const int n = n0 + wn * 64 + ni * 32 + 8 * q + 4 * g;
+          if (n < p.ldc) { p1[q] = *reinterpret_cast<const f32x4*>(crow + n); e[q] = split4_load(erow, n); }
+          else { p1[q] = f32x4{0.f, 0.f, 0.f, 0.f}; e[q] = p1[q]; }
+        }
+#pragma unroll
+        for (int q = 0; q < 4; ++q) {
+          const int nl = wn * 64 + ni * 32 + 8 * q + 4 * g, n = n0 + nl;
+          const f32x4 cv = *reinterpret_cast<const f32x4*>(cvec + nl), dv = *reinterpret_cast<const f32x4*>(cvec + 256 + nl);
+          f32x4 o;
+#pragma unroll
+          for (int k = 0; k < 4; ++k) {
+            const float ek = e[q][k] * (1.f / SPLIT_SCALE_ONE), p2 = acc[mi][ni][4 * q + k] * dq;
+            float v = 0.f;
+            if (n + k < p.N) v = t * ek * ((p1[q][k] - di) * ri + (p2 - dv[k]) * cv[k]);
+            o[k] = v;
+          }
+          if (n < p.ldc) split4_store(crow, n, o * s_out);
+        }
+      }
+    }
+    return;
+  }
 
   const float dq = 1.f / (split_pow2_scale(amax_read(p.amax_a)) * split_pow2_scale(amax_read(p.amax_b)));
   float* __restrict__ cb = p.C + batch * p.c_bs;
@@ -267,17 +392,17 @@
   }
 }
 
-DCN_KNOB(g_gemm3, "Gemm3", 1, "gemm3.hip: the co-attention products on pre-split operands (0 = implicit-GEMM / weight-gradient tiles; + 256 * v = schedule variant v; + 16 * bits = timing ablations, results WRONG)",
+DCN_KNOB(g_gemm3, "Gemm3", 1, "gemm3.hip: the co-attention products on pre-split operands (0 = implicit-GEMM / weight-gradient tiles; + 2 * p = with p set, E and dA come from the streaming passes exp_sums / dA_kernel instead of the products' epilogues; + 256 * v = schedule variant v; + 16 * bits = timing ablations, results WRONG)",
          nullptr, "-DG3_ABL=1", G3_ABL != 0, [](int v) { return (v & 0xF0) != 0; });
 DCN_KNOB(g_gemm3_h1, "H1gemm3", 1, "gemm3.hip: one f16 piece per operand in the bf16 precision modes (0 = both pieces, fp32-accurate co-attention)");
 
-template <bool AT, bool BT, bool H1>
+template <bool AT, bool BT, bool H1, int EPI = G3_EPI_NONE>
 int launch3g_(const G3Params& p, int grid, hipStream_t stream) {
   static DcnPerDeviceFlag attr_once;
   if (attr_once.first()) {
-    (void)hipFuncSetAttribute(reinterpret_cast<const void*>(&gemm3_kernel<AT, BT, H1>), hipFuncAttributeMaxDynamicSharedMemorySize, G3_LDS);
-  }
-  hipLaunchKernelGGL((gemm3_kernel<AT, BT, H1>), dim3(grid), dim3(512), G3_LDS, stream, p);
+    (void)hipFuncSetAttribute(reinterpret_cast<const void*>(&gemm3_kernel<AT, BT, H1, EPI>), hipFuncAttributeMaxDynamicSharedMemorySize, G3_LDS);
+  }
+  hipLaunchKernelGGL((gemm3_kernel<AT, BT, H1, EPI>), dim3(grid), dim3(512), G3_LDS, stream, p);
   return DCN_OK;
 }
 template <bool AT, bool BT>
@@ -305,13 +430,11 @@
   return DCN_OK;
 }
 
-int gemm3_launch(const float* A, int lda, long long a_bs, int at, const float* B, int ldb, long long b_bs, int bt,
-                 float* C, int ldc, long long c_bs, const float* row_scale, long long rs_bs,
-                 int M, int N, int K, int batch, int accumulate, const unsigned* amax_a, const unsigned* amax_b, hipStream_t stream,
-                 unsigned* amax_out) {
+static int g3_params(G3Params& p, const float* A, int lda, long long a_bs, int at, const float* B, int ldb, long long b_bs, int bt,
+                     float* C, int ldc, long long c_bs, int M, int N, int K, const unsigned* amax_a, const unsigned* amax_b) {
   DCN_CHECK_ARG(A && B && C && amax_a && amax_b, "gemm3: null pointer");
   DCN_CHECK_ARG(lda % 4 == 0 && ldb % 4 == 0 && a_bs % 4 == 0 && b_bs % 4 == 0 && (((uintptr_t)A | (uintptr_t)B) & 15) == 0, "gemm3: 16-byte rows");
-  G3Params p{};
+  p = G3Params{};
   p.A = A; p.B = B; p.C = C; p.a_bs = a_bs; p.b_bs = b_bs; p.c_bs = c_bs; p.lda = lda; p.ldb = ldb; p.ldc = ldc;
   p.M = M; p.N = N; p.K = K;
   const int k16 = (K + 15) / 16 * 16;
@@ -319,10 +442,20 @@
   p.a_cols = at ? (M + 7) / 8 * 8 : k16; p.b_cols = bt ? (N + 7) / 8 * 8 : k16;
   DCN_CHECK_ARG(p.a_cols <= lda && p.b_cols <= ldb, "gemm3: rows shorter than the tile reads (lda=%d ldb=%d)", lda, ldb);
   p.tiles_m = cdiv(M, G3_BM); p.tiles_n = cdiv(N, G3_BN);
-  p.row_scale = row_scale; p.rs_bs = rs_bs; p.accumulate = accumulate; p.amax_a = amax_a; p.amax_b = amax_b; p.amax_out = amax_out; p.abl = (g_gemm3 >> 4) & 15; p.var = gemm3_variant();
+  p.amax_a = amax_a; p.amax_b = amax_b; p.abl = (g_gemm3 >> 4) & 15; p.var = gemm3_variant();
+  return DCN_OK;
+}
+
+int gemm3_launch(const float* A, int lda, long long a_bs, int at, const float* B, int ldb, long long b_bs, int bt,
+                 float* C, int ldc, long long c_bs, const float* row_scale, long long rs_bs,
+                 int M, int N, int K, int batch, int accumulate, const unsigned* amax_a, const unsigned* amax_b, hipStream_t stream,
+                 unsigned* amax_out) {
+  G3Params p;
+  int rc = g3_params(p, A, lda, a_bs, at, B, ldb, b_bs, bt, C, ldc, c_bs, M, N, K, amax_a, amax_b);
+  if (rc) return rc;
+  p.row_scale = row_scale; p.rs_bs = rs_bs; p.accumulate = accumulate; p.amax_out = amax_out;
   const int grid = p.tiles_m * p.tiles_n * batch;
   const int pid = prof_begin(40, 2.0 * batch * (double)M * N * K, stream);
-  int rc;
   if (at) rc = bt ? launch3g<true, true>(p, grid, stream) : DCN_ERR_ARG;
   else rc = bt ? launch3g<false, true>(p, grid, stream) : launch3g<false, false>(p, grid, stream);
   prof_end(pid, stream);
@@ -331,6 +464,43 @@
   return DCN_OK;
 }
 
+bool gemm3_fused() { return !(g_gemm3 & 2) && !(g_gemm3_h1 && igemm_precision() == 2); }
+
+int gemm3_launch_exp(const float* A, int lda, long long a_bs, const float* B, int ldb, long long b_bs, float* C, int ldc, long long c_bs,
+                     int M, int N, int K, int batch, const unsigned* amax_a, const unsigned* amax_b, float t, float* rowpart, float* colpart,
+                     hipStream_t stream) {
+  G3Params p;
+  int rc = g3_params(p, A, lda, a_bs, 0, B, ldb, b_bs, 0, C, ldc, c_bs, M, N, K, amax_a, amax_b);
+  if (rc) return rc;
+  DCN_CHECK_ARG(rowpart && ldc % 32 == 0 && ldc >= N && ldc <= p.tiles_n * G3_BN && c_bs % 4 == 0 && ((uintptr_t)C & 15) == 0 &&
+                (!colpart || ((uintptr_t)colpart & 15) == 0), "gemm3 exp epilogue: rows of C are N padded to a multiple of 32, 16-byte aligned");
+  p.t = t; p.rowpart = rowpart; p.colpart = colpart;
+  const int grid = p.tiles_m * p.tiles_n * batch;
+  const int pid = prof_begin(40, 2.0 * batch * (double)M * N * K, stream);
+  if (colpart) launch3g_<false, false, false, G3_EPI_EXP>(p, grid, stream);
+  else launch3g_<false, false, false, G3_EPI_EXP_ROWS>(p, grid, stream);
+  prof_end(pid, stream);
+  DCN_CHECK_LAUNCH("gemm3 exp epilogue");
+  return DCN_OK;
+}
+
+int gemm3_launch_dA(const float* A, int lda, long long a_bs, const float* B, int ldb, long long b_bs, float* C, int ldc, long long c_bs,
+                    int M, int N, int K, int batch, const unsigned* amax_a, const unsigned* amax_b, float t, const float* E,
+                    const float* rinv, const float* cinv, const float* d1, const float* d2, const unsigned* amax_da, hipStream_t stream) {
+  G3Params p;
+  int rc = g3_params(p, A, lda, a_bs, 0, B, ldb, b_bs, 0, C, ldc, c_bs, M, N, K, amax_a, amax_b);
+  if (rc) return rc;
+  DCN_CHECK_ARG(E && rinv && cinv && d1 && d2 && amax_da && ldc % 32 == 0 && ldc >= N && ldc <= p.tiles_n * G3_BN && c_bs % 4 == 0 &&
+                (((uintptr_t)C | (uintptr_t)E) & 15) == 0, "gemm3 dA epilogue: rows of C and E are N padded to a multiple of 32, 16-byte aligned");
+  p.t = t; p.E = E; p.rinv = rinv; p.cinv = cinv; p.d1 = d1; p.d2 = d2; p.amax_da = amax_da;
+  const int grid = p.tiles_m * p.tiles_n * batch;
+  const int pid = prof_begin(40, 2.0 * batch * (double)M * N * K, stream);
+  launch3g_<false, false, false, G3_EPI_DA>(p, grid, stream);
+  prof_end(pid, stream);
+  DCN_CHECK_LAUNCH("gemm3 dA epilogue");
+  return DCN_OK;
+}
+
 extern "C" int dcn_gemm3_supported(int m, int n, int k, int batch) { return gemm3_applicable(m, n, k, batch) ? 1 : 0; }
 
 extern "C" int dcn_gemm3_presplit(const float* src, int ld, int64_t bs, float* dst, int ldd, int64_t bsd, int batch, int rows, int c,
diff --git a/dcnet_amd/csrc/igemm.h b/dcnet_amd/csrc/igemm.h
--- a/dcnet_amd/csrc/igemm.h
+++ b/dcnet_amd/csrc/igemm.h
@@ -87,6 +87,13 @@
                  float* C, int ldc, long long c_bs, const float* row_scale, long long rs_bs,
                  int M, int N, int K, int batch, int accumulate, const unsigned* amax_a, const unsigned* amax_b, hipStream_t stream,
                  unsigned* amax_out = nullptr);
+bool gemm3_fused();
+int gemm3_launch_exp(const float* A, int lda, long long a_bs, const float* B, int ldb, long long b_bs, float* C, int ldc, long long c_bs,
+                     int M, int N, int K, int batch, const unsigned* amax_a, const unsigned* amax_b, float t, float* rowpart, float* colpart,
+                     hipStream_t stream);
+int gemm3_launch_dA(const float* A, int lda, long long a_bs, const float* B, int ldb, long long b_bs, float* C, int ldc, long long c_bs,
+                    int M, int N, int K, int batch, const unsigned* amax_a, const unsigned* amax_b, float t, const float* E,
+                    const float* rinv, const float* cinv, const float* d1, const float* d2, const unsigned* amax_da, hipStream_t stream);
 int igemm_precision();
 extern int g_abl;
 extern int g_wsplit;
```

New measurement: 88.76 clips/s, median of 6. About the same (+0.7%).
